# lukors/kanter_core

Hardware: AMD Instinct MI355X
Metric: node-Mpix/s on 4096x4096 f32x4, 32-node graph (higher is better)
Workload: dtype f32

## Files before the change

bindings/rust/kanter_core_amd_sys.rs:

```rust
#![allow(non_camel_case_types, dead_code)]
use std::os::raw::{c_char, c_void};

pub const KC_OK: i32 = 0;
pub const KC_ERR_GENERIC: i32 = 1;
pub const KC_ERR_CANCELED: i32 = 2;
pub const KC_ERR_IMAGE: i32 = 3;
pub const KC_ERR_INVALID_BUFFER_COUNT: i32 = 4;
pub const KC_ERR_INVALID_NODE_ID: i32 = 5;
pub const KC_ERR_INVALID_NODE_TYPE: i32 = 6;
pub const KC_ERR_INVALID_SLOT_ID: i32 = 7;
pub const KC_ERR_INVALID_SLOT_TYPE: i32 = 8;
pub const KC_ERR_INVALID_EDGE: i32 = 9;
pub const KC_ERR_NO_SLOT_DATA: i32 = 10;
pub const KC_ERR_SLOT_OCCUPIED: i32 = 11;
pub const KC_ERR_SLOT_NOT_OCCUPIED: i32 = 12;
pub const KC_ERR_UNABLE_TO_LOCK: i32 = 13;
pub const KC_ERR_NODE_PROCESSING: i32 = 14;
pub const KC_ERR_POISON: i32 = 15;
pub const KC_ERR_TRY_LOCK: i32 = 16;
pub const KC_ERR_NODE_DIRTY: i32 = 17;
pub const KC_ERR_IO: i32 = 18;
pub const KC_ERR_INVALID_NAME: i32 = 19;
pub const KC_ERR_HIP: i32 = 100;
pub const KC_ERR_NO_DEVICE: i32 = 101;
// ... 216 lines not shown
pub const KC_PARTITION_SPREAD: i32 = 1;
pub const KC_PARTITION_BANDS: i32 = 2;

pub const KC_PLAN_SINGLE: i32 = 0;
pub const KC_PLAN_BRANCHES: i32 = 1;
pub const KC_PLAN_BANDS: i32 = 2;

#[repr(C)] #[derive(Clone, Copy, Debug, PartialEq, Eq)]
pub struct KcBandRange {
    pub y0: i32,
    pub y1: i32,
}

pub const KC_KIND_SOURCE: i32 = 0;
pub const KC_KIND_REPLICATED: i32 = 1;
pub const KC_KIND_COMPUTE: i32 = 2;

#[repr(C)] #[derive(Clone, Copy, Debug, PartialEq, Eq)]
pub struct KcPlacement {
    pub node_id: u32,
    pub rank: i32,
    pub component: i32,
    pub kind: i32,
}

#[repr(C)] #[derive(Clone, Copy, Debug, PartialEq, Eq)]
pub struct KcTransfer {
    pub node_id: u32,
    pub slot_id: u32,
    pub src_rank: i32,
    pub dst_rank: i32,
    pub level: i32,
}

pub const KC_COMM_ID_BYTES: usize = 256;

#[repr(C)] #[derive(Clone, Copy, Debug, PartialEq, Eq)]
pub struct KcBandRows {
    pub node_id: u32,
    pub y0: i32,
    pub y1: i32,
    pub width: u32,
    pub height: u32,
}

#[link(name = "kanter_core_amd")]
extern "C" {
    pub fn kc_init(device_ordinal: i32) -> i32;
    pub fn kc_shutdown() -> i32;
    pub fn kc_is_initialized() -> i32;
    pub fn kc_set_stream(hip_stream: *mut c_void) -> i32;
    pub fn kc_get_stream() -> *mut c_void;
    pub fn kc_sync() -> i32;
    pub fn kc_last_error() -> *const c_char;
    pub fn kc_status_string(status: i32) -> *const c_char;
    pub fn kc_set_fusion(enabled: i32) -> i32;
    pub fn kc_get_fusion() -> i32;
    pub fn kc_set_resize_mode(mode: i32) -> i32;
    pub fn kc_get_resize_mode() -> i32;
    pub fn kc_set_cache_policy(mode: i32) -> i32;
    pub fn kc_get_cache_policy() -> i32;
    pub fn kc_set_option(name: *const c_char, value: i32) -> i32;
    pub fn kc_get_option(name: *const c_char, value: *mut i32) -> i32;
    pub fn kc_resize_upsample_plan(in_n: u32, out_n: u32, filter: i32, eligible: *mut i32, info: *mut i32, rows: *mut f32, cap: usize) -> i32;
    pub fn kc_resize_down2_plan(in_n: u32, out_n: u32, filter: i32, info: *mut i32, left_count: *mut u32, w: *mut f32, wcap: usize, vrec: *mut u32, vcap: usize, hw: *mut f32, hcap: usize) -> i32;
    pub fn kc_stats(bytes_in_use: *mut u64, bytes_cached: *mut u64, kernel_launches: *mut u64) -> i32;
    pub fn kc_stats_algorithmic_bytes(bytes: *mut u64) -> i32;
    pub fn kc_stats_counter(name: *const c_char, value: *mut u64) -> i32;
    pub fn kc_pool_trim() -> i32;
    pub fn kc_set_specialize(mode: i32, after: i32) -> i32;
    pub fn kc_get_specialize() -> i32;
    pub fn kc_specialize_wait() -> i32;
    pub fn kc_specialize_stats(kernels_compiled: *mut u64, compiles_failed: *mut u64, specialized_launches: *mut u64, compiles_pending: *mut u64) -> i32;
    pub fn kc_specialize_compile_check(words: *const u32, n_ops: u32, n_in: u32, start_src: i32, flat: i32, source: *mut c_char, cap: usize) -> i32;
    pub fn kc_specialize_compile_check_mask(words: *const u32, n_ops: u32, n_in: u32, start_src: i32, flat: i32, nt_mask: u32, source: *mut c_char, cap: usize) -> i32;
    pub fn kc_set_chain_quads(quads: i32) -> i32;
    pub fn kc_get_chain_quads() -> i32;
    pub fn kc_specialize_compile_check_upsample(words: *const u32, n_ops: u32, n_in: u32, start_src: i32, taps: u32, wide: i32, source: *mut c_char, cap: usize) -> i32;
    pub fn kc_kernel_cache_set_dir(dir: *const c_char) -> i32;
    pub fn kc_kernel_cache_stats(files_accepted: *mut u64, files_refused: *mut u64, files_written: *mut u64, kernels_loaded: *mut u64) -> i32;
    pub fn kc_kernel_cache_precompile(words: *const u32, n_ops: u32, n_in: u32, start_src: i32, flat: i32, nt_mask: u32, up_taps: u32, up_wide: i32, dir: *const c_char) -> i32;
    pub fn kc_specialize_reset() -> i32;
    pub fn kc_kernel_cache_precompile_packed(words: *const u32, n_ops: u32, n_in: u32, start_src: i32, flat: i32, nt_mask: u32, in_tiers: u32, dir: *const c_char) -> i32;
    pub fn kc_set_pack_sources(mode: i32) -> i32;
    pub fn kc_get_pack_sources() -> i32;
    pub fn kc_set_pack_budget_mb(mb: i32) -> i32;
    pub fn kc_get_pack_budget_mb() -> i32;
    pub fn kc_plane_alloc(width: u32, height: u32, out: *mut *mut KcPlane) -> i32;
    pub fn kc_plane_const(width: u32, height: u32, value: f32, out: *mut *mut KcPlane) -> i32;
    pub fn kc_plane_wrap(device_ptr: *mut c_void, width: u32, height: u32, pitch_bytes: usize, out: *mut *mut KcPlane) -> i32;
    pub fn kc_plane_retain(p: *mut KcPlane) -> i32;
    pub fn kc_plane_release(p: *mut KcPlane) -> i32;
    pub fn kc_plane_size(p: *const KcPlane, width: *mut u32, height: *mut u32) -> i32;
    pub fn kc_plane_is_const(p: *const KcPlane, is_const: *mut i32, value: *mut f32) -> i32;
    pub fn kc_plane_materialize(p: *mut KcPlane) -> i32;
    pub fn kc_plane_device_ptr(p: *mut KcPlane, device_ptr: *mut *mut c_void, pitch_bytes: *mut usize) -> i32;
    pub fn kc_plane_upload_f32(p: *mut KcPlane, host: *const f32, host_pitch_bytes: usize) -> i32;
    pub fn kc_plane_download_f32(p: *mut KcPlane, host: *mut f32, host_pitch_bytes: usize) -> i32;
    pub fn kc_image_gray(p: *mut KcPlane, out: *mut *mut KcImage) -> i32;
    pub fn kc_image_rgba(planes: *const *mut KcPlane, out: *mut *mut KcImage) -> i32;
    pub fn kc_image_retain(img: *mut KcImage) -> i32;
    pub fn kc_image_release(img: *mut KcImage) -> i32;
    pub fn kc_image_is_rgba(img: *const KcImage, is_rgba: *mut i32) -> i32;
    pub fn kc_image_size(img: *const KcImage, size: *mut KcSize) -> i32;
    pub fn kc_image_plane(img: *const KcImage, channel: i32, out: *mut *mut KcPlane) -> i32;
    pub fn kc_image_from_value(size: KcSize, value: f32, rgba: i32, out: *mut *mut KcImage) -> i32;
    pub fn kc_image_as_type(img: *const KcImage, rgba: i32, out: *mut *mut KcImage) -> i32;
    pub fn kc_image_materialize(img: *mut KcImage) -> i32;
    pub fn kc_image_from_u8(host: *const u8, width: u32, height: u32, channels: i32, out: *mut *mut KcImage) -> i32;
    pub fn kc_image_to_u8(img: *mut KcImage, srgb: i32, host_rgba8: *mut u8) -> i32;
    pub fn kc_u8_pipe_create(width: u32, height: u32, channels: i32, depth: i32, out: *mut *mut KcU8Pipe) -> i32;
    pub fn kc_u8_pipe_free(pipe: *mut KcU8Pipe) -> i32;
    pub fn kc_u8_pipe_buffers(pipe: *mut KcU8Pipe, slot: i32, host_in: *mut *mut u8, host_out: *mut *const u8) -> i32;
    pub fn kc_u8_pipe_upload(pipe: *mut KcU8Pipe, slot: i32, out: *mut *mut KcImage) -> i32;
    pub fn kc_u8_pipe_download(pipe: *mut KcU8Pipe, slot: i32, img: *mut KcImage, srgb: i32) -> i32;
    pub fn kc_u8_pipe_wait_download(pipe: *mut KcU8Pipe, slot: i32) -> i32;
    pub fn kc_image_from_f32(host_planes: *const *const f32, n_planes: i32, width: u32, height: u32, out: *mut *mut KcImage) -> i32;
    pub fn kc_image_to_f32(img: *mut KcImage, host_planes: *const *mut f32, n_planes: i32) -> i32;
    pub fn kc_device_image_validate(d: *const KcDeviceImage, extent_bytes: *mut usize) -> i32;
    pub fn kc_image_from_device(src: *const KcDeviceImage, flags: u32, hip_stream: *mut c_void, out: *mut *mut KcImage) -> i32;
    pub fn kc_image_to_device(img: *mut KcImage, dst: *const KcDeviceImage, flags: u32, hip_stream: *mut c_void) -> i32;
    pub fn kc_image_channel_stats(img: *mut KcImage, flags: u32, out: *mut KcChannelStats) -> i32;
    pub fn kc_bc_image_validate(d: *const KcBcImage, extent_bytes: *mut usize) -> i32;
    pub fn kc_bc1_punch_through_block(rgba: *const u8, ref_u8: u32, block: *mut u8) -> i32;
    pub fn kc_image_to_bc(img: *mut KcImage, format: i32, flags: u32, host: *mut u8, host_bytes: usize) -> i32;
    pub fn kc_image_to_bc_device(img: *mut KcImage, dst: *const KcBcImage, flags: u32, hip_stream: *mut c_void) -> i32;
    pub fn kc_mip_level_count(width: u32, height: u32, levels: *mut u32) -> i32;
    pub fn kc_preview_level(width: u32, height: u32, max_extent: u32, level: *mut u32, level_width: *mut u32, level_height: *mut u32) -> i32;
    pub fn kc_image_previews(r: *const KcPreviewRequest, count: u32, flags: u32, host: *mut u8, host_bytes: usize) -> i32;
    pub fn kc_image_previews_device(r: *const KcPreviewRequest, count: u32, flags: u32, device_ptr: *mut c_void, bytes: usize, hip_stream: *mut c_void) -> i32;
    pub fn kc_live_graph_buffer_previews(lg: *mut KcLiveGraph, node_ids: *const u32, slot_ids: *const u32, r: *const KcPreviewRequest, count: u32, flags: u32, host: *mut u8, host_bytes: usize) -> i32;
    pub fn kc_preview_plan(width: u32, height: u32, level: u32, x: u32, y: u32, rect_w: u32, rect_h: u32, out: *mut KcPreviewPlanInfo) -> i32;
    pub fn kc_mip_normal_texel(box_: *const f32, out: *mut f32) -> i32;
    pub fn kc_alpha_ref_threshold(ref_u8: u32, r: *mut f32) -> i32;
    pub fn kc_mip_coverage_target(width: u32, height: u32, covered0: u64, level: u32, target: *mut u64) -> i32;
    pub fn kc_mip_coverage_scale(v: f32, ref_u8: u32, s: *mut f32) -> i32;
    pub fn kc_image_mip_coverage_info(img: *mut KcImage, flags: u32, out: *mut KcMipCoverageLevel, cap: u32, count: *mut u32) -> i32;
    pub fn kc_mip_alpha_weight(a: f32, w: *mut f32) -> i32;
    pub fn kc_mip_alpha_texel(p: *const f32, w: f32, q: *mut f32, known: *mut i32) -> i32;
    pub fn kc_image_build_mips(img: *mut KcImage, flags: u32, levels: *mut *mut KcImage, cap: u32, count: *mut u32) -> i32;
    pub fn kc_bc_mip_layout(width: u32, height: u32, format: i32, levels: *mut u32, offsets: *mut usize, cap: u32, total_bytes: *mut usize) -> i32;
    pub fn kc_image_to_bc_mips(img: *mut KcImage, format: i32, flags: u32, host: *mut u8, host_bytes: usize) -> i32;
    pub fn kc_image_to_bc_mips_device(img: *mut KcImage, format: i32, flags: u32, device_ptr: *mut c_void, bytes: usize, hip_stream: *mut c_void) -> i32;
    pub fn kc_dds_header(width: u32, height: u32, format: i32, flags: u32, levels: u32, out: *mut u8, bytes: *mut usize) -> i32;
    pub fn kc_image_write_dds(img: *mut KcImage, path: *const c_char, format: i32, flags: u32, with_mips: i32) -> i32;
    pub fn kc_mip_unit_normal(rgb: *const f32, u: *mut f32) -> i32;
    pub fn kc_mip_roughness_texel(m: *const f32, r: f32, power: f32, d: *mut f32) -> i32;
    pub fn kc_image_build_roughness_mips(img: *mut KcImage, channel: u32, normals: *mut KcImage, power: f32, flags: u32, levels: *mut *mut KcImage, cap: u32, count: *mut u32) -> i32;
    pub fn kc_image_levels_to_bc_mips(levels: *mut *mut KcImage, count: u32, format: i32, flags: u32, host: *mut u8, host_bytes: usize) -> i32;
    pub fn kc_image_levels_write_dds(levels: *mut *mut KcImage, count: u32, path: *const c_char, format: i32, flags: u32) -> i32;
    pub fn kc_image_distance_field(img: *mut KcImage, channel: u32, ref_u8: u32, spread: u32, flags: u32, out: *mut *mut KcImage) -> i32;
    pub fn kc_sdf_texel(d2: u32, inside: i32, spread: u32, v: *mut f32) -> i32;
    pub fn kc_sdf_cap(spread: u32, cap: *mut u32) -> i32;
    pub fn kc_image_from_bc(host: *const u8, host_bytes: usize, width: u32, height: u32, format: i32, flags: u32, out: *mut *mut KcImage, undecoded_blocks: *mut u64) -> i32;
    pub fn kc_image_from_bc_device(src: *const KcBcImage, flags: u32, hip_stream: *mut c_void, out: *mut *mut KcImage, undecoded_blocks: *mut u64) -> i32;
    pub fn kc_image_bc_compare(img: *mut KcImage, blocks: *const KcBcImage, flags: u32, out: *mut KcBcError) -> i32;
    pub fn kc_image_bc_error(img: *mut KcImage, format: i32, flags: u32, out: *mut KcBcError) -> i32;
    pub fn kc_dds_parse(data: *const u8, bytes: usize, info: *mut KcDdsInfo) -> i32;
    pub fn kc_image_read_dds(path: *const c_char, level: u32, flags: u32, out: *mut *mut KcImage, info: *mut KcDdsInfo) -> i32;
    pub fn kc_image_read_png(path: *const c_char, out: *mut *mut KcImage) -> i32;
    pub fn kc_image_write_png(img: *mut KcImage, path: *const c_char) -> i32;
    pub fn kc_calculate_size(policy: i32, sizes: *const KcSize, n: i32, slot_index: i32, specific: KcSize, out: *mut KcSize) -> i32;
    pub fn kc_resize_image(src: *mut KcImage, size: KcSize, filter: i32, out: *mut *mut KcImage) -> i32;
    pub fn kc_resize_buffers(images: *const *mut KcImage, keys: *const KcEdge, n: i32, edges_sorted: *const KcEdge, n_edges: i32, policy: i32, policy_slot: u32, policy_size: KcSize, filter: i32, out: *mut *mut KcImage) -> i32;
    pub fn kc_mix_process(left: *mut KcImage, right: *mut KcImage, mix_type: i32, out: *mut *mut KcImage) -> i32;
    pub fn kc_separate_rgba_process(input: *mut KcImage, out: *mut *mut KcImage) -> i32;
// ... 87 lines not shown
```

include/kanter_core_amd.h:

```cpp
#ifndef KANTER_CORE_AMD_H
#define KANTER_CORE_AMD_H

#include <stddef.h>
#include <stdint.h>

#ifdef __cplusplus
extern "C" {
#endif

#define KC_API __attribute__((visibility("default")))

typedef enum kc_status {
    KC_OK = 0,
    KC_ERR_GENERIC = 1,
    KC_ERR_CANCELED = 2,
    KC_ERR_IMAGE = 3,
    KC_ERR_INVALID_BUFFER_COUNT = 4,
    KC_ERR_INVALID_NODE_ID = 5,
    KC_ERR_INVALID_NODE_TYPE = 6,
    KC_ERR_INVALID_SLOT_ID = 7,
    KC_ERR_INVALID_SLOT_TYPE = 8,
    KC_ERR_INVALID_EDGE = 9,
    KC_ERR_NO_SLOT_DATA = 10,
    KC_ERR_SLOT_OCCUPIED = 11,
// ... 12 lines not shown
    KC_ERR_UNSUPPORTED = 104
} kc_status;

typedef enum kc_mix_type { KC_MIX_ADD = 0, KC_MIX_SUBTRACT = 1, KC_MIX_MULTIPLY = 2, KC_MIX_DIVIDE = 3, KC_MIX_POW = 4 } kc_mix_type;
typedef enum kc_resize_filter { KC_FILTER_NEAREST = 0, KC_FILTER_TRIANGLE = 1, KC_FILTER_CATMULLROM = 2, KC_FILTER_GAUSSIAN = 3, KC_FILTER_LANCZOS3 = 4 } kc_resize_filter;
typedef enum kc_resize_policy { KC_POLICY_MOST_PIXELS = 0, KC_POLICY_LEAST_PIXELS = 1, KC_POLICY_LARGEST_AXES = 2, KC_POLICY_SMALLEST_AXES = 3, KC_POLICY_SPECIFIC_SLOT = 4, KC_POLICY_SPECIFIC_SIZE = 5 } kc_resize_policy;
typedef enum kc_node_type {
    KC_NODE_INPUT_GRAY = 0, KC_NODE_INPUT_RGBA = 1, KC_NODE_OUTPUT_GRAY = 2, KC_NODE_OUTPUT_RGBA = 3,
    KC_NODE_GRAPH = 4, KC_NODE_IMAGE = 5, KC_NODE_EMBED = 6, KC_NODE_WRITE = 7, KC_NODE_VALUE = 8,
    KC_NODE_MIX = 9, KC_NODE_HEIGHT_TO_NORMAL = 10, KC_NODE_SEPARATE_RGBA = 11, KC_NODE_COMBINE_RGBA = 12
} kc_node_type;
typedef enum kc_node_state { KC_STATE_CLEAN = 0, KC_STATE_DIRTY = 1, KC_STATE_REQUESTED = 2, KC_STATE_PRIORITISED = 3, KC_STATE_PROCESSING = 4, KC_STATE_PROCESSING_DIRTY = 5 } kc_node_state;
typedef enum kc_side { KC_SIDE_INPUT = 0, KC_SIDE_OUTPUT = 1 } kc_side;

typedef struct kc_plane kc_plane;
typedef struct kc_image kc_image;
typedef struct kc_node_graph kc_node_graph;
typedef struct kc_live_graph kc_live_graph;
typedef struct kc_tex_pro kc_tex_pro;
typedef struct kc_partition kc_partition;
typedef struct kc_u8_pipe kc_u8_pipe;

typedef struct kc_size { uint32_t width, height; } kc_size;
typedef struct kc_edge { uint32_t output_id, input_id, output_slot, input_slot; } kc_edge;

typedef struct kc_node_desc {
    uint32_t node_id;
    int32_t node_type;
    int32_t mix_type;
    float value;
    uint32_t embed_id;
    const char *text;
    const kc_node_graph *graph;
    int32_t resize_policy;
    uint32_t policy_slot;
    kc_size policy_size;
    int32_t resize_filter;
} kc_node_desc;

KC_API int kc_init(int device_ordinal);
KC_API int kc_shutdown(void);
KC_API int kc_is_initialized(void);
KC_API int kc_set_stream(void *hip_stream);
KC_API void *kc_get_stream(void);
KC_API int kc_sync(void);
KC_API const char *kc_last_error(void);
KC_API const char *kc_status_string(int status);
KC_API int kc_set_fusion(int enabled);
KC_API int kc_get_fusion(void);
KC_API int kc_set_resize_mode(int mode);
KC_API int kc_get_resize_mode(void);
KC_API int kc_set_cache_policy(int mode);
KC_API int kc_get_cache_policy(void);
KC_API int kc_set_option(const char *name, int value);
KC_API int kc_get_option(const char *name, int *value);
KC_API int kc_resize_upsample_plan(uint32_t in_n, uint32_t out_n, int filter, int *eligible, int32_t info[5], float *rows,
                                   size_t cap);
KC_API int kc_resize_down2_plan(uint32_t in_n, uint32_t out_n, int filter, int32_t info[5], uint32_t *left_count, float *w, size_t wcap,
                                uint32_t *vrec, size_t vcap, float *hw, size_t hcap);
KC_API int kc_stats(uint64_t *bytes_in_use, uint64_t *bytes_cached, uint64_t *kernel_launches);
KC_API int kc_stats_algorithmic_bytes(uint64_t *bytes);
KC_API int kc_stats_counter(const char *name, uint64_t *value);
KC_API int kc_pool_trim(void);
KC_API int kc_set_specialize(int mode, int after);
KC_API int kc_get_specialize(void);
KC_API int kc_specialize_wait(void);
KC_API int kc_specialize_stats(uint64_t *kernels_compiled, uint64_t *compiles_failed, uint64_t *specialized_launches,
                               uint64_t *compiles_pending);
KC_API int kc_specialize_compile_check(const uint32_t *words, uint32_t n_ops, uint32_t n_in, int start_src, int flat,
                                       char *source, size_t cap);
KC_API int kc_specialize_compile_check_mask(const uint32_t *words, uint32_t n_ops, uint32_t n_in, int start_src, int flat,
                                            uint32_t nt_mask, char *source, size_t cap);
KC_API int kc_set_chain_quads(int quads);
KC_API int kc_get_chain_quads(void);
KC_API int kc_specialize_compile_check_upsample(const uint32_t *words, uint32_t n_ops, uint32_t n_in, int start_src, uint32_t taps,
                                                int wide, char *source, size_t cap);
KC_API int kc_kernel_cache_set_dir(const char *dir);
KC_API int kc_kernel_cache_stats(uint64_t *files_accepted, uint64_t *files_refused, uint64_t *files_written, uint64_t *kernels_loaded);
KC_API int kc_kernel_cache_precompile(const uint32_t *words, uint32_t n_ops, uint32_t n_in, int start_src, int flat, uint32_t nt_mask,
                                      uint32_t up_taps, int up_wide, const char *dir);
KC_API int kc_specialize_reset(void);
KC_API int kc_kernel_cache_precompile_packed(const uint32_t *words, uint32_t n_ops, uint32_t n_in, int start_src, int flat,
                                             uint32_t nt_mask, uint32_t in_tiers, const char *dir);
KC_API int kc_set_pack_sources(int mode);
KC_API int kc_get_pack_sources(void);
KC_API int kc_set_pack_budget_mb(int mb);
KC_API int kc_get_pack_budget_mb(void);

KC_API int kc_plane_alloc(uint32_t width, uint32_t height, kc_plane **out);
KC_API int kc_plane_const(uint32_t width, uint32_t height, float value, kc_plane **out);
KC_API int kc_plane_wrap(void *device_ptr, uint32_t width, uint32_t height, size_t pitch_bytes, kc_plane **out);
KC_API int kc_plane_retain(kc_plane *p);
KC_API int kc_plane_release(kc_plane *p);
KC_API int kc_plane_size(const kc_plane *p, uint32_t *width, uint32_t *height);
KC_API int kc_plane_is_const(const kc_plane *p, int *is_const, float *value);
KC_API int kc_plane_materialize(kc_plane *p);
KC_API int kc_plane_device_ptr(kc_plane *p, void **device_ptr, size_t *pitch_bytes);
KC_API int kc_plane_upload_f32(kc_plane *p, const float *host, size_t host_pitch_bytes);
KC_API int kc_plane_download_f32(kc_plane *p, float *host, size_t host_pitch_bytes);

KC_API int kc_image_gray(kc_plane *p, kc_image **out);
KC_API int kc_image_rgba(kc_plane *const planes[4], kc_image **out);
KC_API int kc_image_retain(kc_image *img);
KC_API int kc_image_release(kc_image *img);
KC_API int kc_image_is_rgba(const kc_image *img, int *is_rgba);
KC_API int kc_image_size(const kc_image *img, kc_size *size);
KC_API int kc_image_plane(const kc_image *img, int channel, kc_plane **out);
KC_API int kc_image_from_value(kc_size size, float value, int rgba, kc_image **out);
KC_API int kc_image_as_type(const kc_image *img, int rgba, kc_image **out);
KC_API int kc_image_materialize(kc_image *img);
KC_API int kc_image_from_u8(const uint8_t *host, uint32_t width, uint32_t height, int channels, kc_image **out);
KC_API int kc_image_to_u8(kc_image *img, int srgb, uint8_t *host_rgba8);
KC_API int kc_u8_pipe_create(uint32_t width, uint32_t height, int channels, int depth, kc_u8_pipe **out);
KC_API int kc_u8_pipe_free(kc_u8_pipe *pipe);
KC_API int kc_u8_pipe_buffers(kc_u8_pipe *pipe, int slot, uint8_t **host_in, const uint8_t **host_out);
KC_API int kc_u8_pipe_upload(kc_u8_pipe *pipe, int slot, kc_image **out);
KC_API int kc_u8_pipe_download(kc_u8_pipe *pipe, int slot, kc_image *img, int srgb);
KC_API int kc_u8_pipe_wait_download(kc_u8_pipe *pipe, int slot);
KC_API int kc_image_from_f32(const float *const host_planes[], int n_planes, uint32_t width, uint32_t height, kc_image **out);
KC_API int kc_image_to_f32(kc_image *img, float *const host_planes[], int n_planes);
typedef enum kc_dtype { KC_DTYPE_U8 = 0, KC_DTYPE_U16 = 1, KC_DTYPE_F16 = 2, KC_DTYPE_BF16 = 3, KC_DTYPE_F32 = 4 } kc_dtype;
typedef enum kc_layout { KC_LAYOUT_INTERLEAVED = 0 , KC_LAYOUT_PLANAR = 1  } kc_layout;
typedef struct kc_device_image {
    void *ptr;
    uint32_t width, height;
    int32_t channels;
    int32_t dtype, layout;
    size_t row_pitch_bytes;
    size_t channel_pitch_bytes;
} kc_device_image;
#define KC_DEVICE_SRGB 1u
#define KC_DEVICE_GRAY 2u
KC_API int kc_device_image_validate(const kc_device_image *d, size_t *extent_bytes);
KC_API int kc_image_from_device(const kc_device_image *src, uint32_t flags, void *hip_stream, kc_image **out);
KC_API int kc_image_to_device(kc_image *img, const kc_device_image *dst, uint32_t flags, void *hip_stream);
#define KC_STATS_HISTOGRAM 1u
#define KC_STATS_SRGB 2u
typedef struct kc_channel_stats {
    uint32_t channels;
    uint32_t flags;
    uint64_t pixels;
    float min[4], max[4];
    uint64_t nan_count[4];
    uint64_t histogram[4][256];
} kc_channel_stats;
KC_API int kc_image_channel_stats(kc_image *img, uint32_t flags, kc_channel_stats *out);
typedef enum kc_bc_format { KC_BC1 = 1, KC_BC3 = 3, KC_BC4 = 4, KC_BC5 = 5, KC_BC6H = 95, KC_BC7 = 98 } kc_bc_format;
typedef struct kc_bc_image {
    void *ptr;
    uint32_t width, height;
    int32_t format;
    size_t row_pitch_bytes;
} kc_bc_image;
#define KC_BC_SRGB 1u
#define KC_BC_PUNCH_THROUGH 256u
#define KC_BC_PUNCH_THROUGH_REF(b) (256u | ((uint32_t)(b) << 24))
KC_API int kc_bc_image_validate(const kc_bc_image *d, size_t *extent_bytes);
KC_API int kc_bc1_punch_through_block(const uint8_t rgba[64], uint32_t ref_u8, uint8_t block[8]);
KC_API int kc_image_to_bc(kc_image *img, int format, uint32_t flags, uint8_t *host, size_t host_bytes);
KC_API int kc_image_to_bc_device(kc_image *img, const kc_bc_image *dst, uint32_t flags, void *hip_stream);
#define KC_MIP_PER_LEVEL 2u
#define KC_MIP_NORMALS 32u
#define KC_MIP_COVERAGE 64u
#define KC_MIP_COVERAGE_REF(b) (64u | ((uint32_t)(b) << 24))
#define KC_MIP_ALPHA_WEIGHT 128u
typedef struct kc_mip_coverage_level {
// ... 215 lines not shown
```

kanter_core_amd/__init__.py:

```python
from .api import (Edge, EmbeddedSlotDataId, LiveGraph, MixType, Node, NodeGraph, NodeId, NodeState, NodeType,
                  ResizeFilter, ResizePolicy, Side, Size, SlotData, SlotId, SlotImage, TexProError,
                  TextureProcessor, calculate_size, combine_rgba_process, get_stream, height_to_normal_process,
                  init, is_initialized, mix_process, resize_image, separate_rgba_process, set_fusion, set_stream,
                  shutdown, stats, sync, value_process, set_specialize, get_specialize, specialize_wait,
                  specialize_stats, specialize_compile_check, Partition, PartitionPolicy, NodeKind, set_resize_mode,
                  get_resize_mode, resize_upsample_plan, resize_down2_plan, stats_counter, specialize_compile_check_upsample, specialize_compile_check_mask, set_chain_quads, get_chain_quads, set_pack_sources, get_pack_sources, set_pack_budget_mb, get_pack_budget_mb, set_cache_policy, get_cache_policy, set_option, get_option, comm_unique_id, comm_init,
                  comm_destroy, comm_info, comm_stats, comm_transport, comm_gather_bands, PlanKind, pool_trim, kernel_cache_set_dir, kernel_cache_stats,
                  kernel_cache_precompile, specialize_reset, U8Pipe, device_image_desc, DEVICE_SRGB, DEVICE_GRAY,
                  ChannelStats, STATS_HISTOGRAM, STATS_SRGB, BC_SRGB, BC6H, BC7, BC_BLOCK_BYTES, BC_PUNCH_THROUGH, bc_punch_through_ref, bc1_punch_through_block,
                  MIP_PER_LEVEL, MIP_NORMALS, MIP_COVERAGE, MIP_ALPHA_WEIGHT, mip_alpha_weight, mip_alpha_texel, mip_coverage_ref, MipCoverageLevel, alpha_ref_threshold, mip_coverage_target, mip_coverage_scale, mip_normal_texel, mip_unit_normal, mip_roughness_texel, levels_to_bc_mips, write_dds_levels, mip_level_count, bc_mip_layout, dds_header, BC_GRAY, BC_ALL_MODES, BcError, DdsInfo, dds_parse, preview_level,
                  PREVIEW_SRGB, PreviewPlan, preview_plan, previews, previews_torch, SDF_WRAP, SDF_MAX_SPREAD, sdf_cap, sdf_texel)

__all__ = [n for n in dir() if not n.startswith("_")]
```

kanter_core_amd/_abi.py:

```python
import ctypes as C


KC_OK = 0
KC_ERR_GENERIC = 1
KC_ERR_CANCELED = 2
KC_ERR_IMAGE = 3
KC_ERR_INVALID_BUFFER_COUNT = 4
KC_ERR_INVALID_NODE_ID = 5
KC_ERR_INVALID_NODE_TYPE = 6
KC_ERR_INVALID_SLOT_ID = 7
KC_ERR_INVALID_SLOT_TYPE = 8
KC_ERR_INVALID_EDGE = 9
KC_ERR_NO_SLOT_DATA = 10
KC_ERR_SLOT_OCCUPIED = 11
KC_ERR_SLOT_NOT_OCCUPIED = 12
KC_ERR_UNABLE_TO_LOCK = 13
KC_ERR_NODE_PROCESSING = 14
KC_ERR_POISON = 15
KC_ERR_TRY_LOCK = 16
KC_ERR_NODE_DIRTY = 17
KC_ERR_IO = 18
KC_ERR_INVALID_NAME = 19
KC_ERR_HIP = 100
KC_ERR_NO_DEVICE = 101
# ... 234 lines not shown


class kc_band_range(C.Structure):
    _fields_ = [
        ("y0", C.c_int32),
        ("y1", C.c_int32),
    ]


KC_KIND_SOURCE = 0
KC_KIND_REPLICATED = 1
KC_KIND_COMPUTE = 2


class kc_placement(C.Structure):
    _fields_ = [
        ("node_id", C.c_uint32),
        ("rank", C.c_int32),
        ("component", C.c_int32),
        ("kind", C.c_int32),
    ]


class kc_transfer(C.Structure):
    _fields_ = [
        ("node_id", C.c_uint32),
        ("slot_id", C.c_uint32),
        ("src_rank", C.c_int32),
        ("dst_rank", C.c_int32),
        ("level", C.c_int32),
    ]


KC_COMM_ID_BYTES = 256


class kc_band_rows(C.Structure):
    _fields_ = [
        ("node_id", C.c_uint32),
        ("y0", C.c_int32),
        ("y1", C.c_int32),
        ("width", C.c_uint32),
        ("height", C.c_uint32),
    ]


SIGNATURES = {
    "kc_init": (C.c_int, [C.c_int]),
    "kc_shutdown": (C.c_int, []),
    "kc_is_initialized": (C.c_int, []),
    "kc_set_stream": (C.c_int, [C.c_void_p]),
    "kc_get_stream": (C.c_void_p, []),
    "kc_sync": (C.c_int, []),
    "kc_last_error": (C.c_char_p, []),
    "kc_status_string": (C.c_char_p, [C.c_int]),
    "kc_set_fusion": (C.c_int, [C.c_int]),
    "kc_get_fusion": (C.c_int, []),
    "kc_set_resize_mode": (C.c_int, [C.c_int]),
    "kc_get_resize_mode": (C.c_int, []),
    "kc_set_cache_policy": (C.c_int, [C.c_int]),
    "kc_get_cache_policy": (C.c_int, []),
    "kc_set_option": (C.c_int, [C.c_char_p, C.c_int]),
    "kc_get_option": (C.c_int, [C.c_char_p, C.POINTER(C.c_int)]),
    "kc_resize_upsample_plan": (C.c_int, [C.c_uint32, C.c_uint32, C.c_int, C.POINTER(C.c_int), C.POINTER(C.c_int32), C.c_void_p, C.c_size_t]),
    "kc_resize_down2_plan": (C.c_int, [C.c_uint32, C.c_uint32, C.c_int, C.POINTER(C.c_int32), C.POINTER(C.c_uint32), C.c_void_p, C.c_size_t, C.POINTER(C.c_uint32), C.c_size_t, C.c_void_p, C.c_size_t]),
    "kc_stats": (C.c_int, [C.POINTER(C.c_uint64), C.POINTER(C.c_uint64), C.POINTER(C.c_uint64)]),
    "kc_stats_algorithmic_bytes": (C.c_int, [C.POINTER(C.c_uint64)]),
    "kc_stats_counter": (C.c_int, [C.c_char_p, C.POINTER(C.c_uint64)]),
    "kc_pool_trim": (C.c_int, []),
    "kc_set_specialize": (C.c_int, [C.c_int, C.c_int]),
    "kc_get_specialize": (C.c_int, []),
    "kc_specialize_wait": (C.c_int, []),
    "kc_specialize_stats": (C.c_int, [C.POINTER(C.c_uint64), C.POINTER(C.c_uint64), C.POINTER(C.c_uint64), C.POINTER(C.c_uint64)]),
    "kc_specialize_compile_check": (C.c_int, [C.POINTER(C.c_uint32), C.c_uint32, C.c_uint32, C.c_int, C.c_int, C.c_char_p, C.c_size_t]),
    "kc_specialize_compile_check_mask": (C.c_int, [C.POINTER(C.c_uint32), C.c_uint32, C.c_uint32, C.c_int, C.c_int, C.c_uint32, C.c_char_p, C.c_size_t]),
    "kc_set_chain_quads": (C.c_int, [C.c_int]),
    "kc_get_chain_quads": (C.c_int, []),
    "kc_specialize_compile_check_upsample": (C.c_int, [C.POINTER(C.c_uint32), C.c_uint32, C.c_uint32, C.c_int, C.c_uint32, C.c_int, C.c_char_p, C.c_size_t]),
    "kc_kernel_cache_set_dir": (C.c_int, [C.c_char_p]),
    "kc_kernel_cache_stats": (C.c_int, [C.POINTER(C.c_uint64), C.POINTER(C.c_uint64), C.POINTER(C.c_uint64), C.POINTER(C.c_uint64)]),
    "kc_kernel_cache_precompile": (C.c_int, [C.POINTER(C.c_uint32), C.c_uint32, C.c_uint32, C.c_int, C.c_int, C.c_uint32, C.c_uint32, C.c_int, C.c_char_p]),
    "kc_specialize_reset": (C.c_int, []),
    "kc_kernel_cache_precompile_packed": (C.c_int, [C.POINTER(C.c_uint32), C.c_uint32, C.c_uint32, C.c_int, C.c_int, C.c_uint32, C.c_uint32, C.c_char_p]),
    "kc_set_pack_sources": (C.c_int, [C.c_int]),
    "kc_get_pack_sources": (C.c_int, []),
    "kc_set_pack_budget_mb": (C.c_int, [C.c_int]),
    "kc_get_pack_budget_mb": (C.c_int, []),
    "kc_plane_alloc": (C.c_int, [C.c_uint32, C.c_uint32, C.POINTER(C.c_void_p)]),
    "kc_plane_const": (C.c_int, [C.c_uint32, C.c_uint32, C.c_float, C.POINTER(C.c_void_p)]),
    "kc_plane_wrap": (C.c_int, [C.c_void_p, C.c_uint32, C.c_uint32, C.c_size_t, C.POINTER(C.c_void_p)]),
    "kc_plane_retain": (C.c_int, [C.c_void_p]),
    "kc_plane_release": (C.c_int, [C.c_void_p]),
    "kc_plane_size": (C.c_int, [C.c_void_p, C.POINTER(C.c_uint32), C.POINTER(C.c_uint32)]),
    "kc_plane_is_const": (C.c_int, [C.c_void_p, C.POINTER(C.c_int), C.c_void_p]),
    "kc_plane_materialize": (C.c_int, [C.c_void_p]),
    "kc_plane_device_ptr": (C.c_int, [C.c_void_p, C.POINTER(C.c_void_p), C.POINTER(C.c_size_t)]),
    "kc_plane_upload_f32": (C.c_int, [C.c_void_p, C.c_void_p, C.c_size_t]),
    "kc_plane_download_f32": (C.c_int, [C.c_void_p, C.c_void_p, C.c_size_t]),
    "kc_image_gray": (C.c_int, [C.c_void_p, C.POINTER(C.c_void_p)]),
    "kc_image_rgba": (C.c_int, [C.POINTER(C.c_void_p), C.POINTER(C.c_void_p)]),
    "kc_image_retain": (C.c_int, [C.c_void_p]),
    "kc_image_release": (C.c_int, [C.c_void_p]),
    "kc_image_is_rgba": (C.c_int, [C.c_void_p, C.POINTER(C.c_int)]),
    "kc_image_size": (C.c_int, [C.c_void_p, C.POINTER(kc_size)]),
    "kc_image_plane": (C.c_int, [C.c_void_p, C.c_int, C.POINTER(C.c_void_p)]),
    "kc_image_from_value": (C.c_int, [kc_size, C.c_float, C.c_int, C.POINTER(C.c_void_p)]),
    "kc_image_as_type": (C.c_int, [C.c_void_p, C.c_int, C.POINTER(C.c_void_p)]),
    "kc_image_materialize": (C.c_int, [C.c_void_p]),
    "kc_image_from_u8": (C.c_int, [C.c_void_p, C.c_uint32, C.c_uint32, C.c_int, C.POINTER(C.c_void_p)]),
    "kc_image_to_u8": (C.c_int, [C.c_void_p, C.c_int, C.c_void_p]),
    "kc_u8_pipe_create": (C.c_int, [C.c_uint32, C.c_uint32, C.c_int, C.c_int, C.POINTER(C.c_void_p)]),
    "kc_u8_pipe_free": (C.c_int, [C.c_void_p]),
    "kc_u8_pipe_buffers": (C.c_int, [C.c_void_p, C.c_int, C.POINTER(C.c_void_p), C.POINTER(C.c_void_p)]),
    "kc_u8_pipe_upload": (C.c_int, [C.c_void_p, C.c_int, C.POINTER(C.c_void_p)]),
    "kc_u8_pipe_download": (C.c_int, [C.c_void_p, C.c_int, C.c_void_p, C.c_int]),
    "kc_u8_pipe_wait_download": (C.c_int, [C.c_void_p, C.c_int]),
    "kc_image_from_f32": (C.c_int, [C.POINTER(C.c_void_p), C.c_int, C.c_uint32, C.c_uint32, C.POINTER(C.c_void_p)]),
    "kc_image_to_f32": (C.c_int, [C.c_void_p, C.POINTER(C.c_void_p), C.c_int]),
    "kc_device_image_validate": (C.c_int, [C.POINTER(kc_device_image), C.POINTER(C.c_size_t)]),
    "kc_image_from_device": (C.c_int, [C.POINTER(kc_device_image), C.c_uint32, C.c_void_p, C.POINTER(C.c_void_p)]),
    "kc_image_to_device": (C.c_int, [C.c_void_p, C.POINTER(kc_device_image), C.c_uint32, C.c_void_p]),
    "kc_image_channel_stats": (C.c_int, [C.c_void_p, C.c_uint32, C.POINTER(kc_channel_stats)]),
    "kc_bc_image_validate": (C.c_int, [C.POINTER(kc_bc_image), C.POINTER(C.c_size_t)]),
    "kc_bc1_punch_through_block": (C.c_int, [C.c_void_p, C.c_uint32, C.c_void_p]),
    "kc_image_to_bc": (C.c_int, [C.c_void_p, C.c_int, C.c_uint32, C.c_void_p, C.c_size_t]),
    "kc_image_to_bc_device": (C.c_int, [C.c_void_p, C.POINTER(kc_bc_image), C.c_uint32, C.c_void_p]),
    "kc_mip_level_count": (C.c_int, [C.c_uint32, C.c_uint32, C.POINTER(C.c_uint32)]),
    "kc_preview_level": (C.c_int, [C.c_uint32, C.c_uint32, C.c_uint32, C.POINTER(C.c_uint32), C.POINTER(C.c_uint32), C.POINTER(C.c_uint32)]),
    "kc_image_previews": (C.c_int, [C.POINTER(kc_preview_request), C.c_uint32, C.c_uint32, C.c_void_p, C.c_size_t]),
    "kc_image_previews_device": (C.c_int, [C.POINTER(kc_preview_request), C.c_uint32, C.c_uint32, C.c_void_p, C.c_size_t, C.c_void_p]),
    "kc_live_graph_buffer_previews": (C.c_int, [C.c_void_p, C.POINTER(C.c_uint32), C.POINTER(C.c_uint32), C.POINTER(kc_preview_request), C.c_uint32, C.c_uint32, C.c_void_p, C.c_size_t]),
    "kc_preview_plan": (C.c_int, [C.c_uint32, C.c_uint32, C.c_uint32, C.c_uint32, C.c_uint32, C.c_uint32, C.c_uint32, C.POINTER(kc_preview_plan_info)]),
    "kc_mip_normal_texel": (C.c_int, [C.c_void_p, C.c_void_p]),
    "kc_alpha_ref_threshold": (C.c_int, [C.c_uint32, C.c_void_p]),
    "kc_mip_coverage_target": (C.c_int, [C.c_uint32, C.c_uint32, C.c_uint64, C.c_uint32, C.POINTER(C.c_uint64)]),
    "kc_mip_coverage_scale": (C.c_int, [C.c_float, C.c_uint32, C.c_void_p]),
    "kc_image_mip_coverage_info": (C.c_int, [C.c_void_p, C.c_uint32, C.POINTER(kc_mip_coverage_level), C.c_uint32, C.POINTER(C.c_uint32)]),
    "kc_mip_alpha_weight": (C.c_int, [C.c_float, C.c_void_p]),
    "kc_mip_alpha_texel": (C.c_int, [C.c_void_p, C.c_float, C.c_void_p, C.POINTER(C.c_int)]),
    "kc_image_build_mips": (C.c_int, [C.c_void_p, C.c_uint32, C.POINTER(C.c_void_p), C.c_uint32, C.POINTER(C.c_uint32)]),
    "kc_bc_mip_layout": (C.c_int, [C.c_uint32, C.c_uint32, C.c_int, C.POINTER(C.c_uint32), C.POINTER(C.c_size_t), C.c_uint32, C.POINTER(C.c_size_t)]),
    "kc_image_to_bc_mips": (C.c_int, [C.c_void_p, C.c_int, C.c_uint32, C.c_void_p, C.c_size_t]),
    "kc_image_to_bc_mips_device": (C.c_int, [C.c_void_p, C.c_int, C.c_uint32, C.c_void_p, C.c_size_t, C.c_void_p]),
    "kc_dds_header": (C.c_int, [C.c_uint32, C.c_uint32, C.c_int, C.c_uint32, C.c_uint32, C.c_void_p, C.POINTER(C.c_size_t)]),
    "kc_image_write_dds": (C.c_int, [C.c_void_p, C.c_char_p, C.c_int, C.c_uint32, C.c_int]),
    "kc_mip_unit_normal": (C.c_int, [C.c_void_p, C.c_void_p]),
    "kc_mip_roughness_texel": (C.c_int, [C.c_void_p, C.c_float, C.c_float, C.c_void_p]),
    "kc_image_build_roughness_mips": (C.c_int, [C.c_void_p, C.c_uint32, C.c_void_p, C.c_float, C.c_uint32, C.POINTER(C.c_void_p), C.c_uint32, C.POINTER(C.c_uint32)]),
    "kc_image_levels_to_bc_mips": (C.c_int, [C.POINTER(C.c_void_p), C.c_uint32, C.c_int, C.c_uint32, C.c_void_p, C.c_size_t]),
    "kc_image_levels_write_dds": (C.c_int, [C.POINTER(C.c_void_p), C.c_uint32, C.c_char_p, C.c_int, C.c_uint32]),
    "kc_image_distance_field": (C.c_int, [C.c_void_p, C.c_uint32, C.c_uint32, C.c_uint32, C.c_uint32, C.POINTER(C.c_void_p)]),
    "kc_sdf_texel": (C.c_int, [C.c_uint32, C.c_int, C.c_uint32, C.c_void_p]),
    "kc_sdf_cap": (C.c_int, [C.c_uint32, C.POINTER(C.c_uint32)]),
    "kc_image_from_bc": (C.c_int, [C.c_void_p, C.c_size_t, C.c_uint32, C.c_uint32, C.c_int, C.c_uint32, C.POINTER(C.c_void_p), C.POINTER(C.c_uint64)]),
    "kc_image_from_bc_device": (C.c_int, [C.POINTER(kc_bc_image), C.c_uint32, C.c_void_p, C.POINTER(C.c_void_p), C.POINTER(C.c_uint64)]),
    "kc_image_bc_compare": (C.c_int, [C.c_void_p, C.POINTER(kc_bc_image), C.c_uint32, C.POINTER(kc_bc_error)]),
    "kc_image_bc_error": (C.c_int, [C.c_void_p, C.c_int, C.c_uint32, C.POINTER(kc_bc_error)]),
    "kc_dds_parse": (C.c_int, [C.c_void_p, C.c_size_t, C.POINTER(kc_dds_info)]),
    "kc_image_read_dds": (C.c_int, [C.c_char_p, C.c_uint32, C.c_uint32, C.POINTER(C.c_void_p), C.POINTER(kc_dds_info)]),
    "kc_image_read_png": (C.c_int, [C.c_char_p, C.POINTER(C.c_void_p)]),
    "kc_image_write_png": (C.c_int, [C.c_void_p, C.c_char_p]),
    "kc_calculate_size": (C.c_int, [C.c_int, C.POINTER(kc_size), C.c_int, C.c_int, kc_size, C.POINTER(kc_size)]),
    "kc_resize_image": (C.c_int, [C.c_void_p, kc_size, C.c_int, C.POINTER(C.c_void_p)]),
    "kc_resize_buffers": (C.c_int, [C.POINTER(C.c_void_p), C.POINTER(kc_edge), C.c_int, C.POINTER(kc_edge), C.c_int, C.c_int, C.c_uint32, kc_size, C.c_int, C.POINTER(C.c_void_p)]),
    "kc_mix_process": (C.c_int, [C.c_void_p, C.c_void_p, C.c_int, C.POINTER(C.c_void_p)]),
    "kc_separate_rgba_process": (C.c_int, [C.c_void_p, C.POINTER(C.c_void_p)]),
# ... 87 lines not shown
```

kanter_core_amd/api.py:

```python
import collections
import ctypes as C
import os

import numpy as np

from . import _abi, _lib
from ._lib import kc_edge, kc_node_desc, kc_size

_VARIANT_NAMES = {"KC_ERR_POISON": "PoisonError", "KC_ERR_TRY_LOCK": "TryLockError", "KC_ERR_INVALID_ARG": "InvalidArgument"}
_ERROR_NAMES = {v: _VARIANT_NAMES.get(k, k[len("KC_ERR_"):].title().replace("_", ""))
                for k, v in vars(_abi).items() if k.startswith("KC_ERR_")}


class TexProError(Exception):

    def __init__(self, code, detail=""):
        self.code = code
        self.kind = _ERROR_NAMES.get(code, "Unknown")
        L = _lib.load()
        msg = L.kc_status_string(code).decode()
        super().__init__("%s: %s%s" % (self.kind, msg, (" (" + detail + ")") if detail else ""))

    def __eq__(self, other):
        return isinstance(other, TexProError) and other.code == self.code
# ... 106 lines not shown


def get_option(name):
    v = C.c_int()
    _check(_lib.load().kc_get_option(name.encode(), C.byref(v)))
    return v.value


def resize_upsample_plan(in_n, out_n, filter=None):
    import numpy as np
    L = _lib.load()
    f = ResizeFilter.default() if filter is None else filter
    ok = C.c_int(0)
    info = (C.c_int32 * 5)()
    _check(L.kc_resize_upsample_plan(int(in_n), int(out_n), int(f), C.byref(ok), info, None, 0))
    if not ok.value:
        return None
    ratio, taps, off, b_lo, b_hi = (int(v) for v in info)
    rows = np.zeros(((ratio + b_lo + b_hi), taps), np.float32)
    _check(L.kc_resize_upsample_plan(int(in_n), int(out_n), int(f), C.byref(ok), info,
                                     rows.ctypes.data_as(C.POINTER(C.c_float)), rows.size))
    return dict(ratio=ratio, taps=taps, off=off, b_lo=b_lo, b_hi=b_hi, rows=rows)


def resize_down2_plan(in_n, out_n, filter=None):
    import numpy as np
    L = _lib.load()
    f = ResizeFilter.default() if filter is None else filter
    info = (C.c_int32 * 5)()
    _check(L.kc_resize_down2_plan(int(in_n), int(out_n), int(f), info, None, None, 0, None, 0, None, 0))
    stride, nc, hstride, tile_w, min_count = (int(v) for v in info)
    groups = (out_n + 3) // 4
    lc = np.zeros(2 * out_n, np.uint32)
    w = np.zeros((out_n, stride), np.float32)
    vrec = np.zeros((groups, max(nc, 1), 72), np.uint32)
    hw = np.zeros((out_n, max(hstride, 1)), np.float32)
    _check(L.kc_resize_down2_plan(int(in_n), int(out_n), int(f), info, lc.ctypes.data_as(C.POINTER(C.c_uint32)),
                                  w.ctypes.data_as(C.POINTER(C.c_float)), w.size,
                                  vrec.ctypes.data_as(C.POINTER(C.c_uint32)), vrec.size if nc else 0,
                                  hw.ctypes.data_as(C.POINTER(C.c_float)), hw.size if hstride else 0))
    return dict(stride=stride, nc=nc, hstride=hstride, tile_w=tile_w, min_count=min_count, left=lc[:out_n].copy(),
                count=lc[out_n:].copy(), w=w, vrec=vrec if nc else None, hw=hw if hstride else None)


def set_specialize(mode, after=0):
    _check(_lib.load().kc_set_specialize(int(mode), int(after)))


def get_specialize():
    return _lib.load().kc_get_specialize()


def specialize_wait():
    _check(_lib.load().kc_specialize_wait())


def specialize_stats():
    v = [C.c_uint64() for _ in range(4)]
    _check(_lib.load().kc_specialize_stats(*[C.byref(x) for x in v]))
    return dict(zip(("kernels_compiled", "compiles_failed", "specialized_launches", "compiles_pending"), [x.value for x in v]))


def specialize_compile_check(words, n_in, start_src=0, flat=True):
    arr = (C.c_uint32 * len(words))(*words)
    buf = C.create_string_buffer(1 << 16)
    _check(_lib.load().kc_specialize_compile_check(arr, len(words), int(n_in), int(start_src), int(bool(flat)), buf, len(buf)))
    return buf.value.decode()


def specialize_compile_check_mask(words, n_in, nt_mask, start_src=0, flat=True):
    arr = (C.c_uint32 * len(words))(*words)
    buf = C.create_string_buffer(1 << 17)
    _check(_lib.load().kc_specialize_compile_check_mask(arr, len(words), int(n_in), int(start_src), int(bool(flat)), int(nt_mask),
                                                        buf, len(buf)))
    return buf.value.decode()


def set_chain_quads(quads):
    _check(_lib.load().kc_set_chain_quads(int(quads)))


def get_chain_quads():
    return _lib.load().kc_get_chain_quads()


def set_pack_sources(mode):
    _check(_lib.load().kc_set_pack_sources(int(mode)))


def get_pack_sources():
    return _lib.load().kc_get_pack_sources()


def set_pack_budget_mb(mb):
    _check(_lib.load().kc_set_pack_budget_mb(int(mb)))


def get_pack_budget_mb():
    return _lib.load().kc_get_pack_budget_mb()


def specialize_compile_check_upsample(words, n_in, start_src=0, taps=3, wide=True):
    arr = (C.c_uint32 * len(words))(*words)
    buf = C.create_string_buffer(1 << 17)
    _check(_lib.load().kc_specialize_compile_check_upsample(arr, len(words), int(n_in), int(start_src), int(taps), int(bool(wide)),
                                                            buf, len(buf)))
    return buf.value.decode()


def stats():
    a, b, c = C.c_uint64(), C.c_uint64(), C.c_uint64()
    _check(_lib.load().kc_stats(C.byref(a), C.byref(b), C.byref(c)))
    d = C.c_uint64()
    _check(_lib.load().kc_stats_algorithmic_bytes(C.byref(d)))
    return {"bytes_in_use": a.value, "bytes_cached": b.value, "kernel_launches": c.value, "algorithmic_bytes": d.value}


def kernel_cache_set_dir(path):
    _check(_lib.load().kc_kernel_cache_set_dir(None if path is None else str(path).encode()))


def kernel_cache_stats():
    v = [C.c_uint64() for _ in range(4)]
    _check(_lib.load().kc_kernel_cache_stats(*[C.byref(x) for x in v]))
    return dict(zip(("files_accepted", "files_refused", "files_written", "kernels_loaded"), (x.value for x in v)))


def kernel_cache_precompile(words, n_in, start_src, flat, nt_mask, directory, up_taps=0, up_wide=False, in_tiers=0):
    arr = (C.c_uint32 * len(words))(*words)
    if in_tiers:
        if up_taps:
            raise ValueError("packed inputs: plain chain programs only")
        _check(_lib.load().kc_kernel_cache_precompile_packed(arr, len(words), int(n_in), int(start_src), int(bool(flat)), int(nt_mask),
                                                             int(in_tiers), str(directory).encode()))
        return
    _check(_lib.load().kc_kernel_cache_precompile(arr, len(words), int(n_in), int(start_src), int(bool(flat)), int(nt_mask),
                                                  int(up_taps), int(bool(up_wide)), str(directory).encode()))


def specialize_reset():
    _check(_lib.load().kc_specialize_reset())


def pool_trim():
    _check(_lib.load().kc_pool_trim())


def stats_counter(name):
    v = C.c_uint64()
    _check(_lib.load().kc_stats_counter(name.encode(), C.byref(v)))
    return v.value


class NodeId(int):
    """NodeId(u32), src/node_graph.rs:592-607"""


class SlotId(int):
    """SlotId(u32), src/node_graph.rs:609-624"""


class EmbeddedSlotDataId(int):
    """src/node/embed.rs:13-14"""


class Size:
# ... 1426 lines not shown
```

kanter_core_amd/build.py:

```python
import os
import subprocess
import sys
from concurrent.futures import ThreadPoolExecutor

HERE = os.path.dirname(os.path.abspath(__file__))
CSRC = os.path.join(HERE, "csrc")
OBJ = os.path.join(HERE, "csrc", "build")
LIB = os.path.join(HERE, "libkanter_core_amd.so")
SOURCES = ["chain.hip", "upsample.hip", "resize_tile.hip", "resize_down.hip", "h2n.hip", "u8.hip", "chain1.hip", "down2.hip", "runtime.cpp",
           "ops.cpp", "resize.cpp", "graph.cpp", "json.cpp", "png.cpp", "specialize.cpp", "partition.cpp", "bands.cpp", "comm.cpp", "replay.cpp",
           "u8pipe.cpp", "devimage.hip", "devimage.cpp", "stats.hip", "stats.cpp", "bc.hip", "bc1a.hip", "bc7.hip", "bc6h.hip", "bc.cpp", "mip.hip", "mip_normals.hip", "mip_roughness.hip", "mip_alpha.hip", "mip_coverage.hip", "mip.cpp", "mip_export.cpp", "preview.hip", "preview.cpp", "sdf.hip", "sdf.cpp", "bc_decode.hip",
           "bc_decode.cpp", "bc_modes.hip", "chain_pack.hip", "chain_pack.cpp",
           "c_api.cpp"]
HEADERS = ["kc_internal.hpp", "kc_runtime.hpp", "chain_program.h", "chain_pack.h", "preview_walk.h", "mip_steps.h", os.path.join("..", "..", "include", "kanter_core_amd.h"), "pow_positive.inc",
           "srgb_thresholds.inc", "streaming.h", "bc_blocks.h", "bc_modes.h", "upsample.h", "upsample_chain.inc", "chain_apply.inc", "chain_interp.inc", "resample.inc"]
JIT_TEXTS = [("kJitChainProgramH", "chain_program.h"), ("kJitPowPositiveInc", "pow_positive.inc"), ("kJitUpsampleH", "upsample.h"),
             ("kJitUpsampleChainInc", "upsample_chain.inc"), ("kJitChainPackH", "chain_pack.h")]

FLAGS = ["--offload-arch=gfx950", "-O3", "-std=c++17", "-fPIC", "-fvisibility=hidden", "-fno-fast-math",
         "-ffp-contract=off", "-fhip-fp32-correctly-rounded-divide-sqrt", "-Wall", "-Wno-unused-result"]
DEVICE_FLAGS = ["-mllvm", "-structurizecfg-skip-uniform-regions=1"]
if os.environ.get("KC_HOST_PROFILE"):
    FLAGS = FLAGS + ["-DKC_HOST_PROFILE"]
if os.environ.get("KC_HOST_SAMPLE"):
    FLAGS = FLAGS + ["-DKC_HOST_SAMPLE", "-fno-omit-frame-pointer"]


def _hipcc():
    for cand in (os.environ.get("HIPCC"), "/opt/rocm/bin/hipcc", "hipcc"):
        if cand and (os.path.isabs(cand) and os.path.exists(cand) or not os.path.isabs(cand)):
            return cand
    return "hipcc"


def _stale(target, deps):
    if not os.path.exists(target):
        return True
    t = os.path.getmtime(target)
    return any(os.path.getmtime(d) > t for d in deps)


def object_name(src):
    stem = os.path.splitext(src)[0]
    if src.endswith(".hip") and stem + ".cpp" in SOURCES:
        stem += "_kernels"
    return stem + ".o"


def _write_jit_texts():
    out = os.path.join(OBJ, "jit_texts.cpp")
    parts = ["// generated by kanter_core_amd/build.py from csrc/chain_program.h and csrc/pow_positive.inc -- do not edit\n",
             "namespace kc {\n"]
    for name, fn in JIT_TEXTS:
        with open(os.path.join(CSRC, fn)) as f:
            text = f.read()
        assert ')KCJIT"' not in text
        parts.append('extern const char %s[];\nconst char %s[] = R"KCJIT(\n%s)KCJIT";\n' % (name, name, text))
    parts.append("}  // namespace kc\n")
    new = "".join(parts)
    old = open(out).read() if os.path.exists(out) else None
    if new != old:
        with open(out, "w") as f:
            f.write(new)
    return out


def build(force=False, verbose=False):
    os.makedirs(OBJ, exist_ok=True)
    hipcc = _hipcc()
    hdrs = [os.path.join(CSRC, h) for h in HEADERS]
    jobs = []
    objs = []
    jit = _write_jit_texts()
    jit_o = os.path.join(OBJ, "jit_texts.o")
    objs.append(jit_o)
    if force or _stale(jit_o, [jit]):
        jobs.append([hipcc] + FLAGS + ["-c", jit, "-o", jit_o])
    for src in SOURCES:
        s = os.path.join(CSRC, src)
        o = os.path.join(OBJ, object_name(src))
        objs.append(o)
        if force or _stale(o, [s] + hdrs):
            cmd = [hipcc] + FLAGS + (DEVICE_FLAGS + ["-x", "hip"] if src.endswith(".hip") else []) + ["-c", s, "-o", o]
            jobs.append(cmd)

    def run(cmd):
        if verbose:
            print(" ".join(cmd), flush=True)
        r = subprocess.run(cmd, stdout=subprocess.PIPE, stderr=subprocess.STDOUT, text=True)
        if r.returncode != 0:
            raise RuntimeError("hipcc failed:\n%s\n%s" % (" ".join(cmd), r.stdout))
        return r.stdout

    with ThreadPoolExecutor(max_workers=4) as ex:
        for out in ex.map(run, jobs):
            if verbose and out.strip():
                print(out)
    if force or jobs or _stale(LIB, objs):
        run([hipcc, "--offload-arch=gfx950", "-shared", "-fPIC", "-o", LIB] + objs + ["-lz", "-ldl"])
    populate_kernel_cache(verbose=verbose)
    return LIB


MANIFEST = os.path.join(HERE, "baseline_programs.jsonl")
KERNEL_CACHE = os.path.join(HERE, "kernel_cache")


def populate_kernel_cache(force=False, verbose=False):
    import ctypes as C
    import hashlib
    import json
    if not os.path.exists(MANIFEST) or not os.path.exists(LIB):
        return 0
    with open(MANIFEST) as f:
        text = f.read()
    entries = [json.loads(line) for line in text.splitlines() if line.strip()]
    st = os.stat(LIB)
    stamp = hashlib.sha256(("%s|%d|%d" % (text, st.st_mtime_ns, st.st_size)).encode()).hexdigest()
    stamp_file = os.path.join(KERNEL_CACHE, ".stamp")
    if not force and os.path.exists(stamp_file) and open(stamp_file).read() == stamp:
        return len(entries)
    os.makedirs(KERNEL_CACHE, exist_ok=True)
    for old in os.listdir(KERNEL_CACHE):
        if old.endswith(".kcco"):
            os.remove(os.path.join(KERNEL_CACHE, old))
    L = C.CDLL(LIB)
    L.kc_kernel_cache_precompile.argtypes = [C.POINTER(C.c_uint32), C.c_uint32, C.c_uint32, C.c_int, C.c_int, C.c_uint32, C.c_uint32,
                                             C.c_int, C.c_char_p]
    L.kc_kernel_cache_precompile.restype = C.c_int
    L.kc_kernel_cache_precompile_packed.argtypes = [C.POINTER(C.c_uint32), C.c_uint32, C.c_uint32, C.c_int, C.c_int, C.c_uint32, C.c_uint32,
                                                    C.c_char_p]
    L.kc_kernel_cache_precompile_packed.restype = C.c_int
    L.kc_last_error.restype = C.c_char_p

    def one(e):
        words = (C.c_uint32 * len(e["words"]))(*e["words"])
        if e.get("in_tiers"):
            rc = L.kc_kernel_cache_precompile_packed(words, len(e["words"]), e["n_in"], e["start_src"], e["flat"], e["nt_mask"],
                                                     e["in_tiers"], KERNEL_CACHE.encode())
        else:
            rc = L.kc_kernel_cache_precompile(words, len(e["words"]), e["n_in"], e["start_src"], e["flat"], e["nt_mask"], e["up_taps"],
                                              e["up_wide"], KERNEL_CACHE.encode())
        if rc != 0:
            raise RuntimeError("pre-compiling %s failed (%d): %s" % (e.get("name"), rc, (L.kc_last_error() or b"").decode(errors="replace")))
        if verbose:
            print("pre-compiled", e.get("name"), flush=True)

    with ThreadPoolExecutor(max_workers=4) as ex:
        list(ex.map(one, entries))
    with open(stamp_file, "w") as f:
        f.write(stamp)
    return len(entries)


if __name__ == "__main__":
    print(build(force="--force" in sys.argv, verbose=True))
```

kanter_core_amd/csrc/c_api.cpp:

```cpp
#include <algorithm>
#include <cctype>
#include <climits>
#include <cstdio>
#include <cstdlib>
#include <cstring>
#include <fstream>
#include <sstream>

#include "kc_runtime.hpp"

namespace kc {
const std::string &last_error();
}
using namespace kc;

#define KC_ARG(cond)                                         \
    do {                                                     \
        if (!(cond)) {                                       \
            set_error("invalid argument: " #cond);           \
            return KC_ERR_INVALID_ARG;                       \
        }                                                    \
    } while (0)

typedef std::lock_guard<std::recursive_mutex> Lock;
// ... 347 lines not shown

int kc_specialize_compile_check_mask(const uint32_t *words, uint32_t n_ops, uint32_t n_in, int start_src, int flat, uint32_t nt_mask,
                                     char *source, size_t cap)
try {
    KC_ARG(words && n_ops >= 1 && n_ops <= (uint32_t)KC_CHAIN_MAX_OPS && n_in <= (uint32_t)KC_CHAIN_MAX_IN);
    KC_ARG(start_src >= -1 && start_src < (int)n_in);
    ChainProgram P;
    std::memset(&P, 0, sizeof P);
    P.n_ops = n_ops;
    P.n_in = n_in;
    P.start_src = start_src;
    P.rows = flat ? 1u : 2u;
    P.row_units = 1;
    P.nt_mask = nt_mask;
    for (uint32_t i = 0; i < n_ops; ++i) {
        const uint32_t from = (words[i] >> 8) & 0xffu, level = words[i] >> 16;
        KC_ARG((words[i] & 0xffu) <= CH_SAVE_LOAD && (from <= n_in || (from == (uint32_t)KC_CHAIN_SRC_SAVED && (words[i] & 0xffu) != CH_SAVE_LOAD)));
        KC_ARG(level < (uint32_t)KC_CHAIN_MAX_SAVED && (level == 0 || from == (uint32_t)KC_CHAIN_SRC_SAVED || (words[i] & 0xffu) == CH_SAVE_LOAD));
        ((i & 1u) ? P.step[0][i / 2].b : P.step[0][i / 2].a).word = words[i];
    }
    if (source && cap) {
        const std::string src = specialize_source(P);
        std::snprintf(source, cap, "%s", src.c_str());
    }
    std::string log;
    int s = specialize_compile_only(P, &log);
    if (s != KC_OK) set_error("specialised chain kernel did not compile: " + log);
    return s;
}
KC_CATCH

int kc_set_chain_quads(int quads)
try {
    const int s = specialize_set_chain_quads(quads);
    if (s != KC_OK) set_error("kc_set_chain_quads accepts 0, 1, 2 or 4");
    return s;
}
KC_CATCH

int kc_get_chain_quads(void)
try {
    return specialize_get_chain_quads();
}
catch (...) {
    return 0;
}

int kc_kernel_cache_set_dir(const char *dir)
try {
    Lock lk(ctx().mu);
    return kernel_cache_set_dir(dir);
}
KC_CATCH

int kc_kernel_cache_stats(uint64_t *hits, uint64_t *rejected, uint64_t *written, uint64_t *kernels_loaded)
try {
    kernel_cache_stats(hits, rejected, written, kernels_loaded);
    return KC_OK;
}
KC_CATCH

int kc_kernel_cache_precompile(const uint32_t *words, uint32_t n_ops, uint32_t n_in, int start_src, int flat, uint32_t nt_mask,
                               uint32_t up_taps, int up_wide, const char *dir)
try {
    KC_ARG(words && dir);
    std::string log;
    const int s = kernel_cache_precompile(words, n_ops, n_in, start_src, flat != 0, nt_mask, 0, up_taps, up_wide != 0, dir, &log);
    if (s != KC_OK) set_error("kernel cache: " + log);
    return s;
}
KC_CATCH

int kc_kernel_cache_precompile_packed(const uint32_t *words, uint32_t n_ops, uint32_t n_in, int start_src, int flat, uint32_t nt_mask,
                                      uint32_t in_tiers, const char *dir)
try {
    KC_ARG(words && dir);
    std::string log = "in_tiers: two bits per input plane, 0 to 2, flat programs only";
    const int s = kernel_cache_precompile(words, n_ops, n_in, start_src, flat != 0, nt_mask, in_tiers, 0, false, dir, &log);
    if (s != KC_OK) set_error("kernel cache: " + log);
    return s;
}
KC_CATCH

int kc_set_pack_sources(int mode)
try {
    Lock lk(ctx().mu);
    if (mode < 0 || mode > 2) {
        set_error("kc_set_pack_sources accepts 0, 1 or 2");
        return KC_ERR_INVALID_ARG;
    }
    ctx().pack_sources = mode;
    return KC_OK;
}
KC_CATCH

int kc_get_pack_sources(void)
try {
    return ctx().pack_sources;
}
catch (...) {
    return 0;
}

int kc_set_pack_budget_mb(int mb)
try {
    Lock lk(ctx().mu);
    if (mb < 0) {
        set_error("kc_set_pack_budget_mb accepts 0 and up");
        return KC_ERR_INVALID_ARG;
    }
    ctx().pack_budget_mb = mb;
    return KC_OK;
}
KC_CATCH

int kc_get_pack_budget_mb(void)
try {
    return ctx().pack_budget_mb;
}
catch (...) {
    return 0;
}

int kc_specialize_reset(void)
try {
    Lock lk(ctx().mu);
    if (ctx().stream) (void)hipStreamSynchronize(ctx().stream);
    const int mode = specialize_get_mode();
    specialize_shutdown();
    (void)mode;
    return KC_OK;
}
KC_CATCH

int kc_specialize_compile_check_upsample(const uint32_t *words, uint32_t n_ops, uint32_t n_in, int start_src, uint32_t taps, int wide,
                                         char *source, size_t cap)
try {
    KC_ARG(words && n_ops >= 1 && n_ops <= (uint32_t)KC_CHAIN_MAX_OPS && n_in >= 1 && n_in <= (uint32_t)KC_CHAIN_INTERP_IN);
    KC_ARG(start_src >= -1 && start_src < (int)n_in && (taps == 1 || taps == 3));
    ChainProgram P;
    std::memset(&P, 0, sizeof P);
    P.n_ops = n_ops;
    P.n_in = n_in;
    P.start_src = start_src;
    for (uint32_t i = 0; i < n_ops; ++i) {
        const uint32_t from = words[i] >> 8, code = words[i] & 0xffu;
        KC_ARG(code <= CH_MUL_INV && from <= n_in && code != CH_DIV_L && code != CH_DIV_R && code != CH_POW_L && code != CH_POW_R);
        ((i & 1u) ? P.step[0][i / 2].b : P.step[0][i / 2].a).word = words[i];
    }
    UpsampleArgs U{};
    U.H.taps = U.V.taps = taps;
    U.tile_w = wide ? 1024u : 256u;
    if (source && cap) {
        const std::string src = specialize_source(P, &U);
        std::snprintf(source, cap, "%s", src.c_str());
    }
    std::string log;
    int s = specialize_compile_only(P, &log, &U);
    if (s != KC_OK) set_error("specialised up-sampling kernel did not compile: " + log);
    return s;
}
KC_CATCH

int kc_stats(uint64_t *in_use, uint64_t *cached, uint64_t *launches)
try {
    Context &c = ctx();
// ... 1559 lines not shown
```

kanter_core_amd/csrc/kc_internal.hpp:

```cpp
#pragma once

#include <hip/hip_runtime.h>

#include <atomic>
#include <cstdint>
#include <map>
#include <memory>
#include <mutex>
#include <string>
#include <vector>

#include "../../include/kanter_core_amd.h"
#include "preview_walk.h"

namespace kc {

#include "chain_program.h"
#include "upsample.h"

struct Options {
    int chain1, replay, join, wide, fusion, down2, down2_by_rows, poly2, poly2_min_ratio, resize_mode, resize_tile_w, resize_tile_h;
    int poly_rows, poly2_xcd, down2_xcd, h2n_tiled, cache_policy, cache_budget_mb, nt_force, chain_unroll, max_blocks, tune_cap;
    int upload_ring, link_gbps, hbm_gbps;
};
Options option_defaults();
const Options &options();

struct TapsDev {
    const uint32_t *left;
    const uint32_t *count;
    const float *w;
    uint32_t stride;
};

struct Operand {
    const float *ptr;
    uint32_t pitch;
    float c;
};

struct ChainVariant {
    int k = -1, u = 0, mode = 0;
    bool nt = false;
};
hipError_t launch_chain(const ChainProgram &p, int batch, int mode, int max_blocks, int unroll, hipStream_t s, ChainVariant *var);
inline uint32_t chain_op_word(uint8_t code, int src) { return (uint32_t)code | ((uint32_t)(src + 1) << 8); }
hipError_t launch_fill(float *dst, uint32_t pitch_floats, uint32_t w, uint32_t h, float v, hipStream_t s);
struct Chain1Args {
    const float *start[KC_CHAIN_MAX_BATCH], *operand[KC_CHAIN_MAX_BATCH];
    float *out[KC_CHAIN_MAX_BATCH];
    uint32_t start_pitch[KC_CHAIN_MAX_BATCH], operand_pitch[KC_CHAIN_MAX_BATCH], out_pitch[KC_CHAIN_MAX_BATCH];
    float start_c[KC_CHAIN_MAX_BATCH], operand_c[KC_CHAIN_MAX_BATCH], c[KC_CHAIN_MAX_BATCH];
    uint32_t row_units, rows;
};
hipError_t launch_chain1(const Chain1Args &a, int batch, int code, unsigned nt, hipStream_t s, unsigned *launched_nt);
constexpr uint32_t KC_RESIZE_REG_TAPS = 8;
inline size_t resize_lds_bytes(uint32_t tile_h, uint32_t ncp, uint32_t v_stride, uint32_t tile_w, uint32_t h_stride)
{
    const size_t row = h_stride > KC_RESIZE_REG_TAPS ? (size_t)ncp + (ncp >> 5) + 1u : ncp;
    size_t n = (size_t)tile_h * row + 8u + 2u * tile_h + (size_t)tile_h * v_stride;
    if (h_stride > KC_RESIZE_REG_TAPS) n += 2u * tile_w + (size_t)tile_w * h_stride;
    return n * sizeof(float);
}
#define KC_DOWN_ROW_FLOATS 265u
inline size_t resize_down_lds_bytes(uint32_t tile_h, uint32_t ncp, uint32_t tile_w, uint32_t h_stride)
{
    (void)ncp;
    return ((size_t)tile_h * KC_DOWN_ROW_FLOATS + 2u * tile_w + (size_t)tile_w * (h_stride | 1u)) * sizeof(float);
}
struct ResizePlanes {
    const float *src[4];
    float *dst[4];
    uint32_t spitch[4], dpitch[4];
};
constexpr uint32_t KC_DOWN2_REC = 72, KC_DOWN2_MAX_CHUNKS = 4, KC_DOWN2_SLOTS = 256 + 32;
struct Down2Args {
    const uint32_t *vrec;
    const uint32_t *hleft, *hcount, *strips;
    const float *hw;
    uint32_t nc, hstride;
    uint32_t tile_w, dw, dh;
    uint32_t xcd_per, n_tiles, gy, gy_magic;
    uint32_t by_rows;
};
inline uint32_t down2_cols_per_lane(uint32_t weight_quads) { return weight_quads <= 3 ? 3u : weight_quads == 4 ? 2u : 1u; }
struct XcdOrder {
    uint32_t per, n, gy, magic;
};
inline XcdOrder xcd_order(uint32_t gx, uint32_t gy, bool want)
{
    XcdOrder o{ 0, 0, 0, 0 };
    if (!want || gy < 2) return o;
    const uint64_t n = (uint64_t)gx * gy, magic = ((1ull << 32) + gy - 1) / gy;
    if (n >= (1u << 24) || n * (magic * gy - (1ull << 32)) >= (1ull << 32)) return o;
    o.per = (uint32_t)((n + 7) / 8);
    o.n = (uint32_t)n;
    o.gy = gy;
    o.magic = (uint32_t)magic;
    return o;
}
// ... 299 lines not shown
```

kanter_core_amd/csrc/kc_runtime.hpp:

```cpp
#pragma once

#include <cstring>
#include <deque>
#include <set>
#include <tuple>
#include <type_traits>
#include <unordered_map>
#include <unordered_set>

#include "kc_internal.hpp"

namespace kc {
struct Chain;
struct ChainLink;
}

namespace kc {
#if defined(__SANITIZE_ADDRESS__) || defined(__SANITIZE_THREAD__)
#define KC_NO_OBJECT_POOL 1
#elif defined(__has_feature)
#if __has_feature(address_sanitizer) || __has_feature(thread_sanitizer)
#define KC_NO_OBJECT_POOL 1
#endif
#endif
// ... 346 lines not shown
    uint32_t k, sw, sh, fused;
    bool nt;
    uint32_t last() const { return k + (fused ? fused : 1u); }
};
std::vector<MipStep> mip_plan(uint32_t w, uint32_t h, uint32_t L, bool per_level, uint32_t in0, uint32_t in_below, uint32_t out_planes,
                              const Options &o = options());
int mip_level_count(uint32_t w, uint32_t h, uint32_t *levels);
int preview_level(uint32_t w, uint32_t h, uint32_t max_extent, uint32_t *level, uint32_t *pw, uint32_t *ph);
float mip_const_fold(float c);
void mip_normal_texel(const float box[3], float out[3]);
int image_build_mips(kc_image *img, uint32_t flags, kc_image **levels, uint32_t cap, uint32_t *count);
void mip_unit_normal(const float rgb[3], float u[3]);
float mip_roughness_texel(const float m[3], float r, float power);
int image_build_roughness_mips(kc_image *img, uint32_t channel, kc_image *normals, float power, uint32_t flags, kc_image **levels, uint32_t cap,
                               uint32_t *count);
float mip_alpha_weight(float a);
bool mip_alpha_texel(const float p[3], float w, float q[3]);
int mip_check_alpha_flags(uint32_t flags, const char *who);
constexpr uint32_t kCoverageFlagBits = KC_MIP_COVERAGE | 0xff000000u;
float alpha_ref_threshold(uint32_t ref_u8);
int mip_coverage_target(uint32_t w, uint32_t h, uint64_t covered0, uint32_t level, uint64_t *target);
float mip_coverage_scale(float v, uint32_t ref_u8);
int mip_check_coverage_flags(uint32_t flags, const char *who);
int image_mip_coverage_info(kc_image *img, uint32_t flags, kc_mip_coverage_level *out, uint32_t cap, uint32_t *count);
int bc_mip_layout(uint32_t w, uint32_t h, int format, uint32_t *levels, size_t *offsets, uint32_t cap, size_t *total_bytes);
int image_to_bc_mips(kc_image *img, int format, uint32_t flags, uint8_t *host, size_t host_bytes);
int image_to_bc_mips_device(kc_image *img, int format, uint32_t flags, void *device_ptr, size_t bytes, void *hip_stream);
int dds_header(uint32_t w, uint32_t h, int format, uint32_t flags, uint32_t levels, uint8_t *out, size_t *bytes);
int image_write_dds(kc_image *img, const char *path, int format, uint32_t flags, int with_mips);
int image_levels_to_bc_mips(kc_image *const *levels, uint32_t count, int format, uint32_t flags, uint8_t *host, size_t host_bytes, const char *who);
int image_levels_write_dds(kc_image *const *levels, uint32_t count, const char *path, int format, uint32_t flags);
int preview_plan(uint32_t w, uint32_t h, uint32_t level, uint32_t x, uint32_t y, uint32_t rect_w, uint32_t rect_h, kc_preview_plan_info *out);
int preview_check(const kc_preview_request *r, uint32_t count, uint32_t flags, const void *out, size_t out_bytes, bool images_named, const char *who);
int image_previews(const kc_preview_request *r, kc_image *const *imgs, uint32_t count, uint32_t flags, uint8_t *host, size_t host_bytes, const char *who);
int image_previews_device(const kc_preview_request *r, uint32_t count, uint32_t flags, void *device_ptr, size_t bytes, void *hip_stream);
void preview_release();
int image_channel_stats(kc_image *img, uint32_t flags, kc_channel_stats *out);
uint32_t quant_u8_host(float v);
int stats_buffers(size_t partials_bytes);
void channel_stats_release();
uint32_t sdf_cap(uint32_t spread);
float sdf_texel(uint32_t d2, bool inside, uint32_t spread);
int image_distance_field(kc_image *img, uint32_t channel, uint32_t ref_u8, uint32_t spread, uint32_t flags, kc_image **out);
int calculate_size(int policy, const kc_size *sizes, int n, int slot_index, kc_size specific, kc_size *out);
int mix_process(kc_image *left, kc_image *right, int mix_type, kc_image **out);
int separate_process(kc_image *in, kc_image *out[4]);
int combine_process(kc_image *const in[4], kc_image **out);
int value_process(float v, kc_image **out);
int height_to_normal_process(kc_image *in, kc_image **out);
int height_to_normal_band(kc_image *in_with_halo, uint32_t full_h, kc_image **out);

int build_taps_host(uint32_t in_n, uint32_t out_n, int filter, TapsHost &t);
int resize_image(kc_image *src, kc_size size, int filter, kc_image **out);
int resize_force(kc_plane *p);
int resize_planes_band(kc_plane *const *srcs, int n, int32_t src_y0, uint32_t src_h_full, kc_size dst_full, int32_t a, int32_t b,
                       int filter, kc_plane **outs);
int resize_force_many(kc_plane *const *planes, int n);
int chain_resize_launch(const ChainProgram &P, int batch, int mode, kc_plane *const *sampled, bool *launched);

hipError_t launch_chain_specialized(const ChainProgram &P, int batch, hipStream_t s, bool *launched, uint32_t *nt_mask, uint32_t *quads = nullptr);
uint32_t cache_policy_mask(uint64_t in_bytes, uint64_t out_bytes, uint32_t n_resident, const Options &o = options());
uint32_t chain_cache_policy(const uint32_t *refs, uint32_t n, uint64_t stream_bytes, uint64_t out_bytes);
hipError_t chain_dispatch(ChainProgram &P, int batch, int mode, uint32_t w, uint32_t h, size_t out_pitch_bytes,
                          kc_plane *const (*src)[KC_CHAIN_MAX_IN] = nullptr, const uint32_t *refs = nullptr, uint64_t *packed_saved = nullptr);
uint32_t pack_chain_inputs(const ChainProgram &P, int batch, kc_plane *const (*src)[KC_CHAIN_MAX_IN], const uint32_t *refs, uint32_t w, uint32_t h);
void plane_shadow_drop(kc_plane *p, bool never_again);
uint32_t pack_bytes_per_quad(uint32_t tier);
bool chain_pack_program_ok(const ChainProgram &P);
hipError_t launch_upsample_chain_specialized(const ChainProgram &P, int batch, const UpsampleArgs &U, hipStream_t s, bool *launched);
int specialize_set_mode(int mode, int after);
int specialize_get_mode();
int specialize_set_chain_quads(int quads);
int specialize_get_chain_quads();
void specialize_wait();
void specialize_stats(uint64_t *compiled, uint64_t *failed, uint64_t *launches, uint64_t *pending);
std::string specialize_last_log();
void specialize_shutdown();
std::string specialize_source(const ChainProgram &P, const UpsampleArgs *U = nullptr);
int specialize_compile_only(const ChainProgram &P, std::string *log, const UpsampleArgs *U = nullptr);
int kernel_cache_set_dir(const char *dir);
void kernel_cache_stats(uint64_t *hits, uint64_t *rejected, uint64_t *written, uint64_t *kernels_loaded);
bool kernel_cache_populated();
int kernel_cache_precompile(const uint32_t *words, uint32_t n_ops, uint32_t n_in, int32_t start_src, bool flat, uint32_t nt_mask, uint32_t in_tiers,
                            uint32_t up_taps, bool up_wide, const char *dir, std::string *log);

int u8_pipe_create(uint32_t w, uint32_t h, int channels, int depth, kc_u8_pipe **out);
int u8_pipe_free(kc_u8_pipe *p);
int u8_pipe_buffers(kc_u8_pipe *p, int slot, uint8_t **host_in, const uint8_t **host_out);
int u8_pipe_upload(kc_u8_pipe *p, int slot, kc_image **out);
int u8_pipe_download(kc_u8_pipe *p, int slot, kc_image *img, bool srgb);
int u8_pipe_wait_download(kc_u8_pipe *p, int slot);

int png_read(const std::string &path, std::vector<uint8_t> &px, uint32_t &w, uint32_t &h, int &channels);
int png_write_rgba8(const std::string &path, const uint8_t *px, uint32_t w, uint32_t h);

struct NodeGraph;

struct Node {
    uint32_t node_id = 0;
    int type = KC_NODE_VALUE;
    int mix_type = KC_MIX_ADD;
    float value = 0.0f;
    uint32_t embed_id = 0;
    std::string text;
    std::shared_ptr<NodeGraph> graph;
    int policy = KC_POLICY_MOST_PIXELS;
    uint32_t policy_slot = 0;
    kc_size policy_size{ 0, 0 };
    int filter = KC_FILTER_TRIANGLE;

    bool is_input() const { return type == KC_NODE_INPUT_GRAY || type == KC_NODE_INPUT_RGBA; }
    bool is_output() const { return type == KC_NODE_OUTPUT_GRAY || type == KC_NODE_OUTPUT_RGBA; }
    bool is_source() const { return type == KC_NODE_EMBED || type == KC_NODE_IMAGE || is_input(); }
};

enum SlotType { SLOT_GRAY = 0, SLOT_RGBA = 1, SLOT_GRAY_OR_RGBA = 2 };
struct Slot {
    std::string name;
    uint32_t slot_id;
    int slot_type;
};

struct GraphIndex {
    uint64_t version = ~0ull;
    size_t n_nodes = 0, n_edges = 0;
    std::unordered_map<uint32_t, uint32_t> node_pos;
    std::unordered_map<uint32_t, std::vector<kc_edge>> in_edges;
    std::unordered_map<uint32_t, std::vector<kc_edge>> out_edges;
};

struct NodeGraph {
    std::vector<Node> nodes;
    std::vector<kc_edge> edges;
    uint32_t node_id_counter = 0;
    uint64_t version = 0;
    mutable GraphIndex idx;

    void touch() { ++version; }
    const GraphIndex &index() const;
    bool index_is_current() const;
    void appended_node(bool index_was_current);
    void appended_edge(bool index_was_current);
    void erased_edge(const kc_edge &e, bool index_was_current);
    const std::vector<kc_edge> &edges_into(uint32_t id) const;
    const std::vector<kc_edge> &edges_out_of(uint32_t id) const;

    const Node *find(uint32_t id) const;
    Node *find(uint32_t id);
    uint32_t new_id();
    int add_node(Node n, uint32_t *id);
    int add_node_with_id(Node n);
    int connect(uint32_t on, uint32_t in, uint32_t os, uint32_t is);
    int try_connect(uint32_t on, uint32_t in, uint32_t os, uint32_t is);
    int remove_edge(kc_edge e);
    int remove_node(uint32_t id, std::vector<kc_edge> *removed);
    int disconnect_slot(uint32_t id, int side, uint32_t slot, std::vector<kc_edge> *removed);
    std::vector<uint32_t> get_children(uint32_t id) const;
    std::vector<uint32_t> get_children_recursive(uint32_t id) const;
    std::vector<uint32_t> get_parents(uint32_t id) const;
    std::vector<uint32_t> output_ids() const;
    int rename_output_node(uint32_t id, const std::string &new_name, std::string *old_name);
    std::vector<Slot> input_slots_of_graph() const;
    std::vector<Slot> output_slots_of_graph() const;
};

std::vector<Slot> node_input_slots(const Node &n, bool *unimplemented = nullptr);
std::vector<Slot> node_output_slots(const Node &n, bool *unimplemented = nullptr);
// ... 182 lines not shown
```

kanter_core_amd/csrc/replay.cpp:

```cpp
#include "kc_runtime.hpp"

using namespace kc;

struct kc_live_graph::ReplayEntry {
    uint32_t root = 0;
    uint64_t ghash = 0;
    std::vector<std::pair<uint32_t, int>> pre_state;
    struct Held {
        uint32_t node, slot;
        kc_image *img;
    };
    std::vector<Held> pre_slots;
    std::vector<EmbeddedSlotData> embedded;
    std::vector<std::pair<uint32_t, int>> post_state;
    std::vector<uint32_t> dropped;
    std::vector<uint32_t> changed_ids;
    std::vector<ReplayLaunch> launches;
    uint32_t w = 0, h = 0;
    uint32_t root_slot = 0;
    int n_planes = 0;
    int out_l[4] = { -1, -1, -1, -1 };
    int out_b[4] = { -1, -1, -1, -1 };
    float cval[4] = { 0, 0, 0, 0 };

    ~ReplayEntry()
    {
        for (auto &h : pre_slots) image_release(h.img);
        for (auto &em : embedded) image_release(em.image);
    }
};

namespace kc {

static uint64_t mix64(uint64_t h, uint64_t v)
{
    h ^= v + 0x9E3779B97F4A7C15ull + (h << 6) + (h >> 2);
    return h * 0xBF58476D1CE4E5B9ull;
}

static uint64_t graph_content_hash(const NodeGraph &g)
{
    uint64_t h = 0x243F6A8885A308D3ull;
    h = mix64(h, g.nodes.size());
    for (auto &n : g.nodes) {
        uint32_t vbits;
        std::memcpy(&vbits, &n.value, 4);
        h = mix64(h, ((uint64_t)n.node_id << 32) | (uint32_t)n.type);
        h = mix64(h, ((uint64_t)(uint32_t)n.mix_type << 32) | vbits);
        h = mix64(h, ((uint64_t)n.embed_id << 32) | (uint32_t)n.policy);
        h = mix64(h, ((uint64_t)n.policy_slot << 32) | (uint32_t)n.filter);
        h = mix64(h, ((uint64_t)n.policy_size.width << 32) | n.policy_size.height);
    }
    h = mix64(h, g.edges.size());
    for (auto &e : g.edges) {
        h = mix64(h, ((uint64_t)e.output_id << 32) | e.input_id);
        h = mix64(h, ((uint64_t)e.output_slot << 32) | e.input_slot);
    }
    return h;
}

static bool recordable_type(int t)
{
    return t == KC_NODE_MIX || t == KC_NODE_VALUE || t == KC_NODE_COMBINE_RGBA || t == KC_NODE_SEPARATE_RGBA ||
           t == KC_NODE_OUTPUT_GRAY || t == KC_NODE_OUTPUT_RGBA || t == KC_NODE_EMBED;
}

static size_t slot_count_except(const kc_live_graph &lg, uint32_t node)
{
    size_t n = 0;
    for (auto &kv : lg.slot_datas)
        if (kv.first != node) n += kv.second.size();
    return n;
}

int replay_try(kc_live_graph &lg, uint32_t id, bool *hit)
{
    *hit = false;
    const kc_live_graph::ReplayEntry *e = lg.replay;
    if (!e || e->root != id || lg.use_cache || lg.auto_update || !options().fusion || !options().replay) return KC_OK;
    if (e->pre_state.size() != lg.node_state.size()) return KC_OK;
    for (auto &ps : e->pre_state) {
        auto it = lg.node_state.find(ps.first);
        if (it == lg.node_state.end() || it->second != ps.second) return KC_OK;
    }
    if (slot_count_except(lg, id) != e->pre_slots.size()) return KC_OK;
    for (auto &h : e->pre_slots) {
        const SlotData *sd = lg.find_slot(h.node, h.slot);
        if (!sd || sd->image != h.img) return KC_OK;
    }
    if (lg.embedded.size() != e->embedded.size()) return KC_OK;
    for (size_t i = 0; i < e->embedded.size(); ++i) {
        const EmbeddedSlotData &a = lg.embedded[i], &b = e->embedded[i];
        if (a.image != b.image || a.slot_data_id != b.slot_data_id || a.slot_id != b.slot_id || a.full_h != b.full_h || a.band_y0 != b.band_y0)
            return KC_OK;
    }
    if (graph_content_hash(lg.g) != e->ghash) return KC_OK;

    Context &c = ctx();
    std::vector<kc_plane *> outs(e->launches.size() * KC_CHAIN_MAX_BATCH, nullptr);
    auto drop_outs = [&] {
        for (auto *o : outs) plane_release(o);
    };
    for (size_t li = 0; li < e->launches.size(); ++li) {
        const ReplayLaunch &L = e->launches[li];
        ChainProgram P = L.prog;
        kc_plane *src[KC_CHAIN_MAX_BATCH][KC_CHAIN_MAX_IN] = {};
        for (int b = 0; b < L.batch; ++b) {
            kc_plane *&o = outs[li * KC_CHAIN_MAX_BATCH + b];
            int s = plane_new_mem(L.w, L.h, &o);
            if (s != KC_OK) {
                drop_outs();
                return s;
            }
            P.out[b] = o->dptr;
            P.out_pitch[b] = (uint32_t)(o->pitch / 16);
            for (uint32_t k = 0; k < P.n_in; ++k)
                if (L.in_from[b][k] >= 0) {
                    const kc_plane *res = outs[(size_t)L.in_from[b][k] * KC_CHAIN_MAX_BATCH + L.in_ch[b][k]];
                    P.in[b][k] = res->dptr;
                    P.in_pitch[b][k] = (uint32_t)(res->pitch / 16);
                } else {
                    src[b][k] = L.in_plane[b][k];
                }
        }
        const uint64_t px4 = 4ull * L.w * L.h;
        P.nt_mask = chain_cache_policy(L.in_refs, P.n_in, px4 * L.batch, px4 * L.batch);
        uint64_t packed_saved = 0;
        hipError_t he = chain_dispatch(P, L.batch, L.mode, L.w, L.h, outs[li * KC_CHAIN_MAX_BATCH]->pitch, src, L.in_refs, &packed_saved);
        if (he == hipErrorNotReady) {
            drop_outs();
            return KC_OK;
        }
        if (he != hipSuccess) {
            drop_outs();
            return hip_fail(he, "launch_chain (replay)");
        }
        c.launches++;
        c.alg_bytes += (uint64_t)L.batch * px4 * (P.n_in + 1) - packed_saved;
    }
    c.counters["replayed_evaluations"]++;

    kc_plane *planes[4] = { nullptr, nullptr, nullptr, nullptr };
    std::vector<kc_plane *> consts;
    for (int p = 0; p < e->n_planes; ++p) {
        if (e->out_l[p] >= 0) planes[p] = outs[(size_t)e->out_l[p] * KC_CHAIN_MAX_BATCH + e->out_b[p]];
        else {
            planes[p] = plane_new_const(e->w, e->h, e->cval[p]);
            consts.push_back(planes[p]);
        }
    }
    kc_image *img = image_new(e->n_planes, planes);
    for (auto *q : consts) plane_release(q);
    drop_outs();

    for (uint32_t d : e->dropped) lg.remove_nodes_data(d);
    lg.slot_datas[id].push_back(SlotData{ id, e->root_slot, img });
    for (auto &ps : e->post_state) lg.node_state[ps.first] = ps.second;
    for (uint32_t ch : e->changed_ids) lg.changed.insert(ch);
    *hit = true;
    return KC_OK;
}

struct ReplayRecorder {
    kc_live_graph::ReplayEntry *entry = nullptr;
    ReplayCapture cap;
    uint64_t launches0 = 0;
    std::unordered_set<uint32_t> changed0;
    std::set<const void *> resident0;
    std::set<const kc_plane *> resident_planes;
};

static void note_resident(ReplayRecorder &r, const kc_image *img)
{
    for (int p = 0; p < img->n; ++p)
        if (img->planes[p]->kind == kc_plane::MEM) {
            r.resident0.insert(img->planes[p]->dptr);
            r.resident_planes.insert(img->planes[p]);
        }
}

ReplayRecorder *replay_begin(kc_live_graph &lg, uint32_t id)
{
    Context &c = ctx();
    if (lg.use_cache || lg.auto_update || !c.opt.fusion || !c.opt.replay || c.capture || lg.depth > 0) return nullptr;
    if (lg.g.nodes.size() > 4096) return nullptr;
    auto *r = new ReplayRecorder();
    auto *e = new kc_live_graph::ReplayEntry();
    r->entry = e;
    e->root = id;
    e->ghash = graph_content_hash(lg.g);
    e->pre_state.assign(lg.node_state.begin(), lg.node_state.end());
    for (auto &kv : lg.slot_datas)
        for (auto &sd : kv.second) {
            if (sd.node_id == id) continue;
            image_retain(sd.image);
            e->pre_slots.push_back({ sd.node_id, sd.slot_id, sd.image });
            note_resident(*r, sd.image);
        }
    for (auto &em : lg.embedded) {
        if (em.full_h != 0) {
            delete e;
            delete r;
            return nullptr;
        }
        image_retain(em.image);
        e->embedded.push_back(em);
        note_resident(*r, em.image);
    }
    r->launches0 = c.launches;
    r->changed0 = lg.changed;
    c.capture = &r->cap;
    return r;
}

void replay_end(kc_live_graph &lg, uint32_t id, ReplayRecorder *r, int s)
{
    if (!r) return;
    Context &c = ctx();
    c.capture = nullptr;
    std::unique_ptr<ReplayRecorder> own(r);
    std::unique_ptr<kc_live_graph::ReplayEntry> e(r->entry);
    lg.replay_clear();
    if (s != KC_OK || !r->cap.ok || r->cap.launches.empty() || c.launches - r->launches0 != r->cap.launches.size()) return;
    std::unordered_map<uint32_t, int> pre(e->pre_state.begin(), e->pre_state.end());
    if (pre.size() != lg.node_state.size()) return;
    {
        std::unordered_set<uint32_t> had;
        for (auto &h : e->pre_slots) had.insert(h.node);
        for (auto &n : lg.g.nodes)
            if (!had.count(n.node_id) && !recordable_type(n.type)) return;
    }
    for (auto &kv : lg.node_state) {
        auto it = pre.find(kv.first);
        if (it == pre.end()) return;
        if (it->second != kv.second) {
            const Node *n = lg.g.find(kv.first);
            if (!n || !recordable_type(n->type)) return;
            e->post_state.push_back({ kv.first, kv.second });
        }
    }
    std::unordered_map<uint64_t, kc_image *> before;
    for (auto &h : e->pre_slots) before[((uint64_t)h.node << 32) | h.slot] = h.img;
    std::unordered_set<uint32_t> has_after;
    const SlotData *root_sd = nullptr;
    size_t root_slots = 0;
    for (auto &kv : lg.slot_datas)
        for (auto &sd : kv.second) {
            has_after.insert(sd.node_id);
            if (sd.node_id == id) {
                root_sd = &sd;
                ++root_slots;
                continue;
            }
            auto it = before.find(((uint64_t)sd.node_id << 32) | sd.slot_id);
            if (it == before.end() || it->second != sd.image) return;
        }
    if (!root_sd || root_slots != 1) return;
    std::unordered_set<uint32_t> dropped;
    for (auto &h : e->pre_slots)
        if (!has_after.count(h.node)) dropped.insert(h.node);
    dropped.insert(id);
    for (auto &h : e->pre_slots)
        if (!dropped.count(h.node) && !lg.find_slot(h.node, h.slot)) return;
    e->dropped.assign(dropped.begin(), dropped.end());
    const kc_image *img = root_sd->image;
    ReplayCapture &cap = r->cap;
    e->w = img->w();
    e->h = img->h();
    e->root_slot = root_sd->slot_id;
    e->n_planes = img->n;
    for (int p = 0; p < img->n; ++p) {
        const kc_plane *pl = img->planes[p];
        e->out_l[p] = e->out_b[p] = -1;
        if (pl->kind == kc_plane::CONST) {
            e->cval[p] = pl->cval;
            continue;
        }
        for (size_t li = 0; li < cap.launches.size(); ++li)
            for (int b = 0; b < cap.launches[li].batch; ++b)
                if (cap.launches[li].planes[b] == pl && cap.launches[li].w == img->w() && cap.launches[li].h == img->h()) {
                    e->out_l[p] = (int)li;
                    e->out_b[p] = b;
                }
        if (e->out_l[p] < 0) return;
    }
    for (size_t li = 0; li < cap.launches.size(); ++li) {
        ReplayLaunch &L = cap.launches[li];
        for (int b = 0; b < L.batch; ++b)
            for (uint32_t k = 0; k < L.prog.n_in; ++k) {
                L.in_from[b][k] = L.in_ch[b][k] = -1;
                for (size_t lj = li; lj-- > 0 && L.in_from[b][k] < 0;)
                    for (int bj = 0; bj < cap.launches[lj].batch; ++bj)
                        if (cap.launches[lj].prog.out[bj] == L.prog.in[b][k]) {
                            if (cap.launches[lj].w != L.w || cap.launches[lj].h != L.h) return;
                            L.in_from[b][k] = (int)lj;
                            L.in_ch[b][k] = bj;
                        }
                if (L.in_from[b][k] < 0 && !r->resident0.count(L.prog.in[b][k])) return;
                if (L.in_from[b][k] >= 0 || !r->resident_planes.count(L.in_plane[b][k])) L.in_plane[b][k] = nullptr;
            }
    }
    for (uint32_t ch : lg.changed)
        if (!r->changed0.count(ch)) e->changed_ids.push_back(ch);
    e->launches = std::move(cap.launches);
    lg.replay = e.release();
}

}

void kc_live_graph::replay_clear()
{
    delete replay;
    replay = nullptr;
}
```

kanter_core_amd/csrc/specialize.cpp:

```cpp
#include <dlfcn.h>
#include <sys/stat.h>
#include <unistd.h>

#include <condition_variable>
#include <cstdio>
#include <cstdlib>
#include <cstring>
#include <thread>

#include "kc_runtime.hpp"

namespace kc {

extern const char kJitChainProgramH[];
extern const char kJitPowPositiveInc[];
extern const char kJitUpsampleH[];
extern const char kJitUpsampleChainInc[];
extern const char kJitChainPackH[] __attribute__((weak));

namespace {

typedef struct _hiprtcProgram *hiprtcProgram;
struct Rtc {
    void *lib = nullptr;
    int (*create)(hiprtcProgram *, const char *, const char *, int, const char **, const char **) = nullptr;
    int (*compile)(hiprtcProgram, int, const char **) = nullptr;
    int (*log_size)(hiprtcProgram, size_t *) = nullptr;
    int (*log)(hiprtcProgram, char *) = nullptr;
    int (*code_size)(hiprtcProgram, size_t *) = nullptr;
    int (*code)(hiprtcProgram, char *) = nullptr;
    int (*destroy)(hiprtcProgram *) = nullptr;
    int (*version)(int *, int *) = nullptr;
    bool ok = false;
    bool tried = false;
};

void specialize_stop_at_exit();

Rtc &rtc()
{
    static Rtc r;
    static std::once_flag once;
    std::call_once(once, [] {
        r.tried = true;
        for (const char *name : { "libhiprtc.so", "libhiprtc.so.7", "/opt/rocm/lib/libhiprtc.so" }) {
            r.lib = dlopen(name, RTLD_NOW | RTLD_LOCAL);
            if (r.lib) break;
        }
        if (!r.lib) return;
#define KC_RTC_SYM(field, sym) *(void **)(&r.field) = dlsym(r.lib, sym)
        KC_RTC_SYM(create, "hiprtcCreateProgram");
        KC_RTC_SYM(compile, "hiprtcCompileProgram");
        KC_RTC_SYM(log_size, "hiprtcGetProgramLogSize");
        KC_RTC_SYM(log, "hiprtcGetProgramLog");
        KC_RTC_SYM(code_size, "hiprtcGetCodeSize");
        KC_RTC_SYM(code, "hiprtcGetCode");
        KC_RTC_SYM(destroy, "hiprtcDestroyProgram");
        KC_RTC_SYM(version, "hiprtcVersion");
#undef KC_RTC_SYM
        r.ok = r.create && r.compile && r.log_size && r.log && r.code_size && r.code && r.destroy;
        if (r.ok) std::atexit(specialize_stop_at_exit);
    });
    return r;
}

struct Signature {
    uint32_t n_in = 0, n_ops = 0;
    int32_t start_src = 0;
    bool flat = false;
    uint32_t up_taps = 0;
    bool up_wide = false;
    uint32_t nt_mask = 0;
    uint32_t quads = 1;
    uint32_t in_tiers = 0;
    uint32_t word[KC_CHAIN_MAX_OPS] = {};

    std::string key() const
    {
        std::string k((const char *)&n_in, sizeof n_in);
        k.append((const char *)&n_ops, sizeof n_ops);
        k.append((const char *)&start_src, sizeof start_src);
        k.push_back(flat ? 'f' : 'p');
        k.push_back((char)('0' + up_taps));
        k.push_back(up_wide ? 'w' : 'n');
        k.append((const char *)&nt_mask, sizeof nt_mask);
        k.append((const char *)word, sizeof(uint32_t) * n_ops);
        if (quads > 1) {
            k.push_back('q');
            k.push_back((char)('0' + quads));
        }
        if (in_tiers) {
            k.push_back('t');
            k.append((const char *)&in_tiers, sizeof in_tiers);
        }
        return k;
    }
};

constexpr uint32_t kQuadsWarm = 2, kQuadsMaxOps = 16;
std::atomic<int> g_chain_quads{ 0 };

uint32_t chain_quads_for(const Signature &s, uint64_t total_units)
{
    if (s.up_taps || !s.flat || s.n_in < 1 || s.n_ops > kQuadsMaxOps || total_units > 0xF0000000ull) return 1;
    bool plain = false;
    for (uint32_t k = 0; k < s.n_in; ++k) plain |= !(s.nt_mask & KC_CHAIN_NT_BIT(k));
    if (!plain || !s.nt_mask) return 1;
    for (uint32_t i = 0; i < s.n_ops; ++i) {
        const uint32_t code = s.word[i] & 0xffu;
        if (code == CH_DIV_L || code == CH_DIV_R || code == CH_POW_L || code == CH_POW_R) return 1;
    }
    const int forced = g_chain_quads.load(std::memory_order_relaxed);
    return forced ? (uint32_t)forced : kQuadsWarm;
}

bool pack_program_ok(const ChainProgram &P)
{
    if (P.n_ops < 1 || P.n_ops > kQuadsMaxOps || P.n_in < 1 || P.rows != 1) return false;
    for (uint32_t i = 0; i < P.n_ops; ++i) {
        const uint32_t code = ((i & 1u) ? P.step[0][i / 2].b.word : P.step[0][i / 2].a.word) & 0xffu;
        if (code == CH_DIV_L || code == CH_DIV_R || code == CH_POW_L || code == CH_POW_R) return false;
    }
    return true;
}

Signature signature_of(const ChainProgram &P, const UpsampleArgs *U = nullptr)
{
    Signature s;
    s.n_in = P.n_in;
    s.n_ops = P.n_ops;
    s.start_src = P.start_src;
    s.flat = U ? false : P.rows == 1;
    {
        uint32_t valid = 0x100u;
        for (uint32_t k = 0; k < (U ? P.n_in - 1u : P.n_in); ++k) valid |= KC_CHAIN_NT_BIT(k);
        s.nt_mask = P.nt_mask & valid;
    }
    if (U) {
        s.up_taps = U->H.taps;
        s.up_wide = U->tile_w == 1024;
    }
    for (uint32_t i = 0; i < P.n_ops; ++i) s.word[i] = (i & 1u) ? P.step[0][i / 2].b.word : P.step[0][i / 2].a.word;
    if (!U && s.flat) s.in_tiers = P.n_in >= 16 ? P.in_tiers : P.in_tiers & ((1u << (2 * P.n_in)) - 1u);
    s.quads = chain_quads_for(s, (uint64_t)P.rows * P.row_units);
    return s;
}

static int spec_wg()
{
    static int wg = [] {
        int v = 256;
        if (const char *e = std::getenv("KC_SPEC_WG")) {
            const int x = std::atoi(e);
            if (x == 64 || x == 128 || x == 256 || x == 512 || x == 1024) v = x;
        }
        return v;
    }();
    return wg;
}

std::string kernel_name(const Signature &s)
{
    uint32_t h = 2166136261u;
    for (unsigned char c : s.key()) h = (h ^ c) * 16777619u;
    char buf[32];
    std::snprintf(buf, sizeof buf, s.up_taps ? "kc_upchain_%08x" : "kc_chain_%08x", h);
    return buf;
}

static const char kPackedF4[] = R"KCF4(typedef float raw4 __attribute__((ext_vector_type(4)));
typedef float f2 __attribute__((ext_vector_type(2)));
typedef unsigned long long __attribute__((may_alias)) rec64;
static __device__ __forceinline__ f2 pk_sub(f2 a, f2 b)
{
    f2 d;
    asm("v_pk_add_f32 %0, %1, %2 neg_lo:[0,1] neg_hi:[0,1]" : "=v"(d) : "v"(a), "v"(b));
    return d;
}
struct kconst {
    rec64 rec;  // { word, c }
    __device__ __forceinline__ operator float() const { return __builtin_bit_cast(float, (unsigned int)(rec >> 32)); }
    __device__ __forceinline__ f2 minus(f2 b) const
    {
        f2 d;
        asm("v_pk_add_f32 %0, %1, %2 op_sel_hi:[0,1] neg_lo:[0,1] neg_hi:[0,1]" : "=v"(d) : "s"(rec >> 32), "v"(b));
        return d;
    }
};
struct f4 {
    f2 lo, hi;
    f4() = default;
    __device__ __forceinline__ f4(float x, float y, float z, float w) : lo{ x, y }, hi{ z, w } {}
    __device__ __forceinline__ f4(f2 l, f2 h) : lo(l), hi(h) {}
    __device__ __forceinline__ f4(raw4 v) : lo(v.xy), hi(v.zw) {}
    __device__ __forceinline__ raw4 raw() const { return raw4{ lo.x, lo.y, hi.x, hi.y }; }
};
static __device__ __forceinline__ f4 operator+(f4 a, f4 b) { return f4(a.lo + b.lo, a.hi + b.hi); }
static __device__ __forceinline__ f4 operator*(f4 a, f4 b) { return f4(a.lo * b.lo, a.hi * b.hi); }
static __device__ __forceinline__ f4 operator-(f4 a, f4 b) { return f4(pk_sub(a.lo, b.lo), pk_sub(a.hi, b.hi)); }
static __device__ __forceinline__ f4 operator-(kconst c, f4 b) { return f4(c.minus(b.lo), c.minus(b.hi)); }
static __device__ __forceinline__ f4 operator/(f4 a, f4 b) { return f4(a.raw() / b.raw()); }
struct StepRecView { kconst c; };
struct StepPairView { StepRecView a, b; };
struct StepTableView {
    const ChainStepPair *p;
    __device__ __forceinline__ StepPairView operator[](unsigned int i) const
    {
        const rec64 *q = reinterpret_cast<const rec64 *>(p + i);
        return StepPairView{ { { q[0] } }, { { q[1] } } };
    }
};
)KCF4";

static std::string step_expr(const Signature &s, uint32_t i, const char *in_prefix, const char *in_suffix)
{
    const uint32_t code = s.word[i] & 0xffu, from = (s.word[i] >> 8) & 0xffu, level = (s.word[i] >> 16) & 3u;
    char c[48], x[96];
    std::snprintf(c, sizeof c, "pp[%u].%c.c", i / 2, (i & 1u) ? 'b' : 'a');
    if (from == 0)
        std::snprintf(x, sizeof x, "f4{ %s, %s, %s, %s }", c, c, c, c);
    else if (from == (uint32_t)KC_CHAIN_SRC_SAVED)
        std::snprintf(x, sizeof x, "saved%u", level);
    else
        std::snprintf(x, sizeof x, "%s%u%s", in_prefix, from - 1, in_suffix);
    switch (code) {
    case CH_SAVE_LOAD: return "(saved" + std::to_string(level) + " = acc, " + x + ")";
    case CH_ADD: return std::string("acc + ") + x;
    case CH_SUB_L: return std::string("acc - ") + x;
    case CH_SUB_R: return std::string(x) + " - acc";
    case CH_MUL: return std::string("acc * ") + x;
    case CH_DIV_L: return std::string("acc / ") + x;
    case CH_DIV_R: return std::string(x) + " / acc";
    case CH_POW_L: return std::string("pow4(acc, ") + x + ", pow_tab)";
    case CH_POW_R: return std::string("pow4(") + x + ", acc, pow_tab)";
    case CH_ADD_INV: return std::string(c) + " - (acc + " + x + ")";
    case CH_SUBL_INV: return std::string(c) + " - (acc - " + x + ")";
    case CH_SUBR_INV: return std::string(c) + " - (" + x + " - acc)";
    case CH_MUL_INV: return std::string(c) + " - (acc * " + x + ")";
    default: return std::string();
    }
}

static std::string generate_up(const Signature &s)
{
    std::string src;
    src.reserve(32768);
    src += "namespace kc {\n";
    src += kJitChainProgramH;
    src += kJitUpsampleH;
// ... 28 lines not shown
                  kernel_name(s).c_str(), s.n_in, s.up_taps, KC_UPSAMPLE_ROWS, s.up_wide ? "true" : "false", s.nt_mask);
    src += buf;
    return src;
}

static std::string load_expr(const Signature &s, uint32_t k, const std::string &at)
{
    const uint32_t tier = KC_CHAIN_TIER(s.in_tiers, k);
    const bool nt = (s.nt_mask & KC_CHAIN_NT_BIT(k)) != 0;
    const std::string in = "P.in[b][" + std::to_string(k) + "]";
    std::string ptr;
    if (tier == (uint32_t)KC_PACK_FIX24)
        ptr = "reinterpret_cast<const pack_u3a *>(reinterpret_cast<const char *>(" + in + ") + (unsigned long long)(" + at + ") * 12u)";
    else if (tier == (uint32_t)KC_PACK_U8)
        ptr = "&reinterpret_cast<const unsigned int *>(" + in + ")[" + at + "]";
    else
        ptr = "&reinterpret_cast<const raw4 *>(" + in + ")[" + at + "]";
    const std::string v = nt ? "__builtin_nontemporal_load(" + ptr + ")" : "*(" + ptr + ")";
    return tier == (uint32_t)KC_PACK_FIX24 ? "pack_decode_fix24(" + v + ")" : tier == (uint32_t)KC_PACK_U8 ? "pack_decode_u8(" + v + ")" : v;
}

static std::string generate_quads(const Signature &s, int SPEC_WG)
{
    std::string src;
    char buf[320];
    std::snprintf(buf, sizeof buf,
                  "    const unsigned int n = P.rows * P.row_units;\n"
                  "    const unsigned int idx = blockIdx.x * %uu + threadIdx.x;\n    if (idx >= n) return;\n",
                  s.quads * (uint32_t)SPEC_WG);
    src += buf;
    for (uint32_t u = 0; u < s.quads; ++u) {
        if (u == 0)
            src += "    const unsigned int at0 = idx;\n";
        else {
            std::snprintf(buf, sizeof buf, "    const unsigned int at%u = idx + %uu < n ? idx + %uu : n - 1u;\n", u, u * SPEC_WG, u * SPEC_WG);
            src += buf;
        }
        for (uint32_t k = 0; k < s.n_in; ++k) {
            if (KC_CHAIN_TIER(s.in_tiers, k)) {
                src += "    const f4 in" + std::to_string(k) + "_" + std::to_string(u) + " = " + load_expr(s, k, "at" + std::to_string(u)) + ";\n";
                continue;
            }
            if (s.nt_mask & KC_CHAIN_NT_BIT(k))
                std::snprintf(buf, sizeof buf, "    const f4 in%u_%u = __builtin_nontemporal_load(&reinterpret_cast<const raw4 *>(P.in[b][%u])[at%u]);\n", k, u, k, u);
            else
                std::snprintf(buf, sizeof buf, "    const f4 in%u_%u = reinterpret_cast<const raw4 *>(P.in[b][%u])[at%u];\n", k, u, k, u);
            src += buf;
        }
    }
    src += "    const StepTableView pp{ P.step[b] };\n";
    for (uint32_t u = 0; u < s.quads; ++u) {
        char suffix[8];
        std::snprintf(suffix, sizeof suffix, "_%u", u);
        std::snprintf(buf, sizeof buf, "    f4 out%u;\n    {\n", u);
        src += buf;
        if (s.start_src < 0)
            src += "        f4 acc = f4{ P.start_c[b], P.start_c[b], P.start_c[b], P.start_c[b] };\n";
        else {
            std::snprintf(buf, sizeof buf, "        f4 acc = in%d%s;\n", s.start_src, suffix);
            src += buf;
        }
        src += "        f4 saved0 = acc, saved1 = acc, saved2 = acc;\n";
        for (uint32_t i = 0; i < s.n_ops; ++i) {
            const std::string e = step_expr(s, i, "in", suffix);
            if (e.empty()) return std::string();
            src += "        acc = " + e + ";\n";
        }
        std::snprintf(buf, sizeof buf, "        out%u = acc;\n    }\n", u);
        src += buf;
    }
    for (uint32_t u = 0; u < s.quads; ++u) {
        std::snprintf(buf, sizeof buf, "    if (idx + %uu < n) ", u * SPEC_WG);
        src += u ? buf : "    ";
        std::snprintf(buf, sizeof buf,
                      s.nt_mask & 0x100u ? "__builtin_nontemporal_store(out%u.raw(), &reinterpret_cast<raw4 *>(P.out[b])[idx + %uu]);\n"
                                         : "reinterpret_cast<raw4 *>(P.out[b])[idx + %uu] = out%u.raw();\n",
                      s.nt_mask & 0x100u ? u : u * SPEC_WG, s.nt_mask & 0x100u ? u * SPEC_WG : u);
        src += buf;
    }
    src += "}\n";
    return src;
}

std::string generate(const Signature &s)
{
    if (s.up_taps) return generate_up(s);
    const int SPEC_WG = spec_wg();
    bool pow = false;
    for (uint32_t i = 0; i < s.n_ops; ++i) pow |= (s.word[i] & 0xffu) == CH_POW_L || (s.word[i] & 0xffu) == CH_POW_R;
    std::string src;
    src.reserve(16384);
    src += "namespace kc {\n";
    src += kJitChainProgramH;
    src += kPackedF4;
    if (s.in_tiers) {
        const char *pack_text = kJitChainPackH;
        if (!pack_text) return std::string();
        src += pack_text;
    }
    if (pow) {
        src += kJitPowPositiveInc;
        src += "static __device__ __noinline__ float pow_general(float a, float b) { return (float)pow((double)a, (double)b); }\n"
               "static __device__ __forceinline__ float kc_powf(float a, float b, const PowCtx &pw)\n"
               "{\n"
               "    if (a > 0.0f && a < __builtin_inff() && __builtin_fabsf(b) < __builtin_inff()) return pow_positive(a, b, pw);\n"
               "    return pow_general(a, b);\n"
               "}\n"
               "static __device__ __forceinline__ f4 pow4(f4 a, f4 b, const PowCtx &t) { return f4{ kc_powf(a.lo.x, b.lo.x, t), kc_powf(a.lo.y, b.lo.y, t), kc_powf(a.hi.x, b.hi.x, t), kc_powf(a.hi.y, b.hi.y, t) }; }\n";
    }
    src += "}  // namespace kc\nusing namespace kc;\n";
    char buf[256];
    std::snprintf(buf, sizeof buf, "extern \"C\" __global__ __launch_bounds__(%d) void %s(const ChainProgram P)\n{\n", SPEC_WG,
                  kernel_name(s).c_str());
    src += buf;
    if (pow) src += "    __shared__ double pow_lds[KC_POW_TABLE_DOUBLES];\n    const PowCtx pow_tab = pow_setup(pow_lds);\n";
    src += "    const unsigned int b = blockIdx.y;\n";
    if (s.quads > 1) {
        const std::string body = generate_quads(s, SPEC_WG);
        return body.empty() ? body : src + body;
    }
    std::snprintf(buf, sizeof buf, "    const unsigned int idx = blockIdx.x * %du + threadIdx.x;\n", SPEC_WG);
    src += buf;
    src += "    if (idx >= P.rows * P.row_units) return;\n";
    if (s.flat)
        src += "    const unsigned int row = 0u, col = idx;\n";
    else
        src += "    const unsigned int row = idx / P.row_units, col = idx - row * P.row_units;\n";
    for (uint32_t k = 0; k < s.n_in; ++k) {
        if (KC_CHAIN_TIER(s.in_tiers, k)) {
            src += "    const f4 in" + std::to_string(k) + " = " + load_expr(s, k, "col") + ";\n";
            continue;
        }
        if (s.nt_mask & KC_CHAIN_NT_BIT(k))
            std::snprintf(buf, sizeof buf, "    const f4 in%u = __builtin_nontemporal_load(&reinterpret_cast<const raw4 *>(P.in[b][%u])[row * P.in_pitch[b][%u] + col]);\n", k, k, k);
        else
            std::snprintf(buf, sizeof buf, "    const f4 in%u = reinterpret_cast<const raw4 *>(P.in[b][%u])[row * P.in_pitch[b][%u] + col];\n", k, k, k);
        src += buf;
    }
    src += "    const StepTableView pp{ P.step[b] };\n";
    if (s.start_src < 0)
        src += "    f4 acc = f4{ P.start_c[b], P.start_c[b], P.start_c[b], P.start_c[b] };\n";
    else {
        std::snprintf(buf, sizeof buf, "    f4 acc = in%d;\n", s.start_src);
        src += buf;
    }
    src += "    f4 saved0 = acc, saved1 = acc, saved2 = acc;\n";
    for (uint32_t i = 0; i < s.n_ops; ++i) {
        const std::string e = step_expr(s, i, "in", "");
        if (e.empty()) return std::string();
        src += "    acc = " + e + ";\n";
    }
    if (s.nt_mask & 0x100u)
        src += "    __builtin_nontemporal_store(acc.raw(), &reinterpret_cast<raw4 *>(P.out[b])[row * P.out_pitch[b] + col]);\n}\n";
    else
        src += "    reinterpret_cast<raw4 *>(P.out[b])[row * P.out_pitch[b] + col] = acc.raw();\n}\n";
    return src;
}

static const char *const kCompileOpts[] = { "--gpu-architecture=gfx950", "-O3", "-ffp-contract=off", "-fno-fast-math",
                                            "-fhip-fp32-correctly-rounded-divide-sqrt" };
constexpr int kNumCompileOpts = (int)(sizeof kCompileOpts / sizeof *kCompileOpts);

uint64_t fnv64(const void *data, size_t n, uint64_t h = 1469598103934665603ull)
{
    const unsigned char *p = (const unsigned char *)data;
    for (size_t i = 0; i < n; ++i) h = (h ^ p[i]) * 1099511628211ull;
    return h;
}

// ... 198 lines not shown
    return true;
}

struct Entry {
    enum State { COUNTING, QUEUED, READY, FAILED } state = COUNTING;
    uint32_t sightings = 0;
    Signature sig;
    hipModule_t module = nullptr;
    hipFunction_t fn = nullptr;
};

struct Spec {
    std::mutex mu;
    std::condition_variable cv, idle_cv;
    std::map<std::string, Entry> cache;
    std::unordered_map<uint64_t, std::pair<std::string, Entry *>> by_hash;
    std::deque<std::string> queue;
    std::thread worker;
    bool worker_running = false, stopping = false;
    int busy = 0;
    std::atomic<int> mode{ 1 };
    uint32_t after = 2;
    int device = -1;
    uint64_t compiled = 0, failed = 0, launches = 0, loaded_from_disk = 0;
    std::string last_log;

    void stop()
    {
        {
            std::lock_guard<std::mutex> lk(mu);
            stopping = true;
            for (auto &key : queue) {
                auto it = cache.find(key);
                if (it != cache.end() && it->second.state == Entry::QUEUED) {
                    it->second.state = Entry::COUNTING;
                    it->second.sightings = 0;
                }
            }
            queue.clear();
        }
        cv.notify_all();
        idle_cv.notify_all();
        if (worker.joinable()) worker.join();
        std::lock_guard<std::mutex> lk(mu);
        worker_running = false;
        stopping = false;
    }
};

Spec &spec()
{
    static Spec *s = new Spec();
    return *s;
}

void specialize_stop_at_exit() { spec().stop(); }

bool compile_entry(const Signature &sig, hipModule_t *module, hipFunction_t *fn, std::string *log, bool disk_only = false)
{
    const std::string src = generate(sig);
    if (src.empty()) {
        *log = "unknown step code";
        return false;
    }
    std::vector<char> code;
    if (disk_load(sig, src, code)) {
        if (load_code(sig, code, module, fn, log)) return true;
        std::lock_guard<std::mutex> lk(disk().mu);
        disk().hits--;
        disk().rejected++;
    }
    if (disk_only) {
        *log = "not in the kernel cache";
        return false;
    }
    if (!rtc_compile(src, code, log)) return false;
    if (!load_code(sig, code, module, fn, log)) return false;
    disk_store(sig, src, code);
    if (const char *m = std::getenv("KC_KERNEL_CACHE_MANIFEST")) {
        if (FILE *f = std::fopen(m, "a")) {
            std::fprintf(f, "{\"name\": \"%s\", \"n_in\": %u, \"start_src\": %d, \"flat\": %d, \"nt_mask\": %u, \"up_taps\": %u, \"up_wide\": %d, \"words\": [",
                         kernel_name(sig).c_str(), sig.n_in, sig.start_src, sig.flat ? 1 : 0, sig.nt_mask, sig.up_taps, sig.up_wide ? 1 : 0);
            for (uint32_t k = 0; k < sig.n_ops; ++k) std::fprintf(f, "%s%u", k ? ", " : "", sig.word[k]);
            if (sig.in_tiers) std::fprintf(f, "], \"in_tiers\": %u}\n", sig.in_tiers);
            else std::fprintf(f, "]}\n");
            std::fclose(f);
        }
    }
    return true;
}

void finish(Spec &S, const std::string &key, bool ok, hipModule_t m, hipFunction_t f, const std::string &log, bool from_disk = false)
{
    auto it = S.cache.find(key);
    if (it == S.cache.end()) {
        if (ok) (void)hipModuleUnload(m);
        return;
    }
    if (ok) {
        it->second.module = m;
        it->second.fn = f;
        it->second.state = Entry::READY;
        if (from_disk) S.loaded_from_disk++;
        else S.compiled++;
    } else {
        it->second.state = Entry::FAILED;
        S.failed++;
        S.last_log = log;
    }
}

void worker_main()
{
    Spec &S = spec();
    if (S.device >= 0) (void)hipSetDevice(S.device);
    std::unique_lock<std::mutex> lk(S.mu);
    for (;;) {
        S.cv.wait(lk, [&] { return S.stopping || !S.queue.empty(); });
        if (S.stopping) return;
        const std::string key = S.queue.front();
        S.queue.pop_front();
        auto it = S.cache.find(key);
        if (it == S.cache.end()) continue;
        const Signature sig = it->second.sig;
        S.busy++;
        lk.unlock();
        hipModule_t m = nullptr;
        hipFunction_t f = nullptr;
        std::string log;
        const uint64_t hits0 = disk_hits();
        const bool ok = compile_entry(sig, &m, &f, &log);
        const bool from_disk = ok && disk_hits() != hits0;
        lk.lock();
        S.busy--;
        finish(S, key, ok, m, f, log, from_disk);
        S.idle_cv.notify_all();
    }
}

}

static uint64_t signature_hash(const Signature &s)
{
    uint64_t h = 1469598103934665603ull;
    auto mix = [&](uint64_t v) { h = (h ^ v) * 1099511628211ull; };
    mix(s.n_in);
    mix(s.n_ops);
    mix((uint64_t)(int64_t)s.start_src);
    mix(s.flat ? 1 : 0);
    mix(s.up_taps);
    mix(s.up_wide ? 1 : 0);
    mix(s.nt_mask);
    mix(s.quads);
    mix(s.in_tiers);
    for (uint32_t i = 0; i < s.n_ops; ++i) mix(s.word[i]);
    return h;
}

static bool same_signature(const Signature &a, const Signature &b)
{
    return a.n_in == b.n_in && a.n_ops == b.n_ops && a.start_src == b.start_src && a.flat == b.flat && a.up_taps == b.up_taps &&
           a.up_wide == b.up_wide && a.nt_mask == b.nt_mask && a.quads == b.quads && a.in_tiers == b.in_tiers &&
           std::memcmp(a.word, b.word, sizeof(uint32_t) * a.n_ops) == 0;
}

static hipFunction_t spec_lookup(const Signature &sig)
{
    Spec &S = spec();
    if (S.mode.load(std::memory_order_relaxed) == 0) return nullptr;
    const uint64_t h = signature_hash(sig);
    {
        std::lock_guard<std::mutex> fast(S.mu);
        auto it = S.by_hash.find(h);
        if (it != S.by_hash.end() && it->second.second->state == Entry::READY && same_signature(it->second.second->sig, sig))
            return it->second.second->fn;
    }
    const std::string key = sig.key();
    std::unique_lock<std::mutex> lk(S.mu);
    if (S.mode == 2) {
        auto it = S.cache.find(key);
        if (it != S.cache.end() && it->second.state == Entry::QUEUED)
            S.idle_cv.wait(lk, [&] { return S.cache[key].state != Entry::QUEUED || !S.worker_running; });
    }
    Entry &e = S.cache[key];
    if (e.state == Entry::READY) {
        e.sig = sig;
        S.by_hash[h] = { key, &e };
        return e.fn;
    }
    if (e.state != Entry::COUNTING) return nullptr;
    e.sightings++;
    if (e.sightings == 1 && S.mode == 1) {
        hipModule_t m = nullptr;
        hipFunction_t f = nullptr;
        std::string log;
        e.sig = sig;
        if (compile_entry(sig, &m, &f, &log, true)) {
            e.module = m;
            e.fn = f;
            e.state = Entry::READY;
            S.loaded_from_disk++;
            S.by_hash[h] = { key, &e };
            return f;
        }
    }
    if (S.mode == 1 && e.sightings < S.after) return nullptr;
    e.sig = sig;
    if (S.mode == 2) {
        e.state = Entry::QUEUED;
        lk.unlock();
        hipModule_t m = nullptr;
        hipFunction_t f = nullptr;
        std::string log;
        const uint64_t hits0 = disk_hits();
        const bool ok = compile_entry(sig, &m, &f, &log);
        const bool from_disk = ok && disk_hits() != hits0;
        lk.lock();
        finish(S, key, ok, m, f, log, from_disk);
        return ok ? f : nullptr;
    }
    e.state = Entry::QUEUED;
    S.queue.push_back(key);
    if (!S.worker_running) {
        S.device = ctx().device;
        S.stopping = false;
        S.worker = std::thread(worker_main);
        S.worker_running = true;
    }
    lk.unlock();
    S.cv.notify_one();
    return nullptr;
}

hipError_t launch_chain_specialized(const ChainProgram &P, int batch, hipStream_t s, bool *launched, uint32_t *nt_mask, uint32_t *quads)
{
    *launched = false;
    if (P.n_ops < 1 || P.n_ops > (uint32_t)KC_CHAIN_MAX_OPS || P.n_in > (uint32_t)KC_CHAIN_MAX_IN) return hipSuccess;
    const uint64_t total = (uint64_t)P.rows * P.row_units;
    if (total == 0 || total > 0xFFFFFFFFull) return hipSuccess;
    const Signature sig = signature_of(P);
    hipFunction_t fn = spec_lookup(sig);
    if (!fn) return hipSuccess;
    size_t size = sizeof(ChainProgram);
    const int SPEC_WG = spec_wg();
    void *extra[] = { HIP_LAUNCH_PARAM_BUFFER_POINTER, (void *)&P, HIP_LAUNCH_PARAM_BUFFER_SIZE, &size, HIP_LAUNCH_PARAM_END };
    const uint64_t per_block = (uint64_t)SPEC_WG * sig.quads;
    const unsigned gx = (unsigned)((total + per_block - 1) / per_block);
    hipError_t e = hipModuleLaunchKernel(fn, gx, (unsigned)batch, 1, SPEC_WG, 1, 1, 0, s, nullptr, extra);
    if (e == hipSuccess) {
        *launched = true;
        if (nt_mask) *nt_mask = sig.nt_mask;
        if (quads) *quads = sig.quads;
        std::lock_guard<std::mutex> lk(spec().mu);
        spec().launches++;
    }
    return e;
}

bool chain_pack_program_ok(const ChainProgram &P) { return pack_program_ok(P); }

hipError_t launch_upsample_chain_specialized(const ChainProgram &P, int batch, const UpsampleArgs &U, hipStream_t s, bool *launched)
{
    *launched = false;
    if (P.n_ops < 1 || P.n_ops > (uint32_t)KC_CHAIN_MAX_OPS || P.n_in < 1 || P.n_in > (uint32_t)KC_CHAIN_INTERP_IN) return hipSuccess;
    if (!upsample_args_ok(U, batch) || (U.H.taps != 1 && U.H.taps != 3)) return hipSuccess;
    if (U.H.ratio == 2) return hipSuccess;
    hipFunction_t fn = spec_lookup(signature_of(P, &U));
    if (!fn) return hipSuccess;
    struct alignas(16) Params {
        ChainProgram P;
        UpsampleArgs U;
    };
    static_assert(sizeof(ChainProgram) % alignof(UpsampleArgs) == 0, "the second kernel argument follows the first without padding");
    static thread_local Params params;
    params.P = P;
    params.U = U;
    size_t size = sizeof(Params);
    void *extra[] = { HIP_LAUNCH_PARAM_BUFFER_POINTER, (void *)&params, HIP_LAUNCH_PARAM_BUFFER_SIZE, &size, HIP_LAUNCH_PARAM_END };
    const dim3 grid = upsample_grid(U, batch);
    hipError_t e = hipModuleLaunchKernel(fn, grid.x, grid.y, grid.z, 256, 1, 1, (unsigned)upsample_lds_bytes(U), s, nullptr, extra);
    if (e == hipSuccess) {
        *launched = true;
        std::lock_guard<std::mutex> lk(spec().mu);
        spec().launches++;
    }
    return e;
}

int specialize_set_mode(int mode, int after)
{
    Spec &S = spec();
    if (mode < 0 || mode > 2) return KC_ERR_INVALID_ARG;
    {
        std::lock_guard<std::mutex> lk(S.mu);
        S.mode.store(mode);
        if (after >= 1) S.after = (uint32_t)after;
    }
    if (mode == 0) S.stop();
    return KC_OK;
}

int specialize_get_mode()
{
    Spec &S = spec();
    return S.mode.load();
}

void specialize_wait()
{
    Spec &S = spec();
    std::unique_lock<std::mutex> lk(S.mu);
    S.idle_cv.wait(lk, [&] { return S.stopping || (S.queue.empty() && S.busy == 0); });
}

void specialize_stats(uint64_t *compiled, uint64_t *failed, uint64_t *launches, uint64_t *pending)
{
    Spec &S = spec();
    std::lock_guard<std::mutex> lk(S.mu);
    if (compiled) *compiled = S.compiled;
    if (failed) *failed = S.failed;
    if (launches) *launches = S.launches;
    if (pending) *pending = S.queue.size() + (uint64_t)S.busy;
}

std::string specialize_last_log()
{
    Spec &S = spec();
    std::lock_guard<std::mutex> lk(S.mu);
    return S.last_log;
}

void specialize_shutdown()
{
    Spec &S = spec();
    S.stop();
    std::lock_guard<std::mutex> lk(S.mu);
    for (auto &kv : S.cache)
        if (kv.second.module) (void)hipModuleUnload(kv.second.module);
    S.by_hash.clear();
    S.cache.clear();
}

int specialize_set_chain_quads(int quads)
{
    if (quads != 0 && quads != 1 && quads != 2 && quads != 4) return KC_ERR_INVALID_ARG;
    g_chain_quads.store(quads);
    return KC_OK;
}

int specialize_get_chain_quads() { return g_chain_quads.load(); }

std::string specialize_source(const ChainProgram &P, const UpsampleArgs *U) { return generate(signature_of(P, U)); }

int specialize_compile_only(const ChainProgram &P, std::string *log, const UpsampleArgs *U)
{
    if (!rtc().ok) {
        *log = "libhiprtc not available";
        return KC_ERR_UNSUPPORTED;
    }
    const std::string src = generate(signature_of(P, U));
    if (src.empty()) return KC_ERR_GENERIC;
    std::vector<char> code;
    return rtc_compile(src, code, log) ? KC_OK : KC_ERR_GENERIC;
}

int kernel_cache_set_dir(const char *dir)
{
    DiskCache &d = disk();
    std::lock_guard<std::mutex> lk(d.mu);
    resolve_dirs_locked(d, dir && *dir ? dir : nullptr);
    return KC_OK;
}

void kernel_cache_stats(uint64_t *hits, uint64_t *rejected, uint64_t *written, uint64_t *kernels_loaded)
{
    {
        DiskCache &d = disk();
        std::lock_guard<std::mutex> lk(d.mu);
        if (hits) *hits = d.hits;
        if (rejected) *rejected = d.rejected;
        if (written) *written = d.written;
    }
    Spec &S = spec();
    std::lock_guard<std::mutex> lk(S.mu);
    if (kernels_loaded) *kernels_loaded = S.loaded_from_disk;
}

bool kernel_cache_populated()
{
    DiskCache &d = disk();
    std::vector<std::string> dirs;
    {
        std::lock_guard<std::mutex> lk(d.mu);
        if (!d.resolved) resolve_dirs_locked(d, nullptr);
        dirs = d.read_dirs;
        if (dirs.empty()) return false;
        if (d.hits) return true;
    }
    static std::map<std::string, bool> seen;
    for (auto &dir : dirs) {
        auto it = seen.find(dir);
        if (it == seen.end()) {
            bool any = false;
            std::string probe = dir + "/.populated";
            any = access(probe.c_str(), R_OK) == 0;
            it = seen.emplace(dir, any).first;
        }
        if (it->second) return true;
    }
    return false;
}

int kernel_cache_precompile(const uint32_t *words, uint32_t n_ops, uint32_t n_in, int32_t start_src, bool flat, uint32_t nt_mask, uint32_t in_tiers,
                            uint32_t up_taps, bool up_wide, const char *dir, std::string *log)
{
    if (in_tiers && (!flat || up_taps || (n_in < 16 && in_tiers >> (2 * n_in)))) return KC_ERR_INVALID_ARG;
    for (uint32_t k = 0; k < n_in; ++k)
        if (KC_CHAIN_TIER(in_tiers, k) == 3u) return KC_ERR_INVALID_ARG;
    if (!words || n_ops < 1 || n_ops > (uint32_t)KC_CHAIN_MAX_OPS || n_in > (uint32_t)KC_CHAIN_MAX_IN || !dir || !*dir) return KC_ERR_INVALID_ARG;
    Signature sig;
    sig.n_in = n_in;
    sig.n_ops = n_ops;
    sig.start_src = start_src;
    sig.flat = flat;
    sig.nt_mask = nt_mask;
    sig.up_taps = up_taps;
    sig.up_wide = up_wide;
    sig.in_tiers = in_tiers;
    for (uint32_t i = 0; i < n_ops; ++i) sig.word[i] = words[i];
    sig.quads = chain_quads_for(sig, 0);
    const std::string src = generate(sig);
    if (src.empty()) {
        *log = "unknown step code";
        return KC_ERR_INVALID_ARG;
    }
    std::vector<char> code;
    if (!rtc_compile(src, code, log)) return rtc().ok ? KC_ERR_GENERIC : KC_ERR_UNSUPPORTED;
    if (!make_dirs(dir) || !disk_store_in(dir, sig, src, code)) {
        *log = std::string("cannot write into ") + dir;
        return KC_ERR_IO;
    }
    if (FILE *f = std::fopen((std::string(dir) + "/.populated").c_str(), "w")) std::fclose(f);
    return KC_OK;
}

}
```

Before: 7.132 million.

## Fuse replayed chain launches into tapped kernels that store intermediate outputs

Adds a tapped chain kernel that runs a short per-pixel op chain once and writes every needed intermediate result (taps) to its output plane. Replay groups consecutive chain launches into one such launch, avoiding separate kernel launches and the re-read of intermediate planes from memory. The feature is on by default and needs runtime-compiled kernels. It adds replay-plan complexity and falls back to the old path when pitches or program shapes don't fit.

```diff
diff --git a/bindings/rust/kanter_core_amd_sys.rs b/bindings/rust/kanter_core_amd_sys.rs
--- a/bindings/rust/kanter_core_amd_sys.rs
+++ b/bindings/rust/kanter_core_amd_sys.rs
@@ -322,6 +322,10 @@
     pub fn kc_kernel_cache_precompile(words: *const u32, n_ops: u32, n_in: u32, start_src: i32, flat: i32, nt_mask: u32, up_taps: u32, up_wide: i32, dir: *const c_char) -> i32;
     pub fn kc_specialize_reset() -> i32;
     pub fn kc_kernel_cache_precompile_packed(words: *const u32, n_ops: u32, n_in: u32, start_src: i32, flat: i32, nt_mask: u32, in_tiers: u32, dir: *const c_char) -> i32;
+    pub fn kc_set_replay_taps(on: i32) -> i32;
+    pub fn kc_get_replay_taps() -> i32;
+    pub fn kc_specialize_compile_check_taps(words: *const u32, n_ops: u32, n_in: u32, start_src: i32, nt_mask: u32, tap_mask: u32, source: *mut c_char, cap: usize) -> i32;
+    pub fn kc_kernel_cache_precompile_taps(words: *const u32, n_ops: u32, n_in: u32, start_src: i32, nt_mask: u32, tap_mask: u32, dir: *const c_char) -> i32;
     pub fn kc_set_pack_sources(mode: i32) -> i32;
     pub fn kc_get_pack_sources() -> i32;
     pub fn kc_set_pack_budget_mb(mb: i32) -> i32;
diff --git a/include/kanter_core_amd.h b/include/kanter_core_amd.h
--- a/include/kanter_core_amd.h
+++ b/include/kanter_core_amd.h
@@ -118,6 +118,12 @@
 KC_API int kc_specialize_reset(void);
 KC_API int kc_kernel_cache_precompile_packed(const uint32_t *words, uint32_t n_ops, uint32_t n_in, int start_src, int flat,
                                              uint32_t nt_mask, uint32_t in_tiers, const char *dir);
+KC_API int kc_set_replay_taps(int on);
+KC_API int kc_get_replay_taps(void);
+KC_API int kc_specialize_compile_check_taps(const uint32_t *words, uint32_t n_ops, uint32_t n_in, int start_src, uint32_t nt_mask,
+                                            uint32_t tap_mask, char *source, size_t cap);
+KC_API int kc_kernel_cache_precompile_taps(const uint32_t *words, uint32_t n_ops, uint32_t n_in, int start_src, uint32_t nt_mask,
+                                           uint32_t tap_mask, const char *dir);
 KC_API int kc_set_pack_sources(int mode);
 KC_API int kc_get_pack_sources(void);
 KC_API int kc_set_pack_budget_mb(int mb);
diff --git a/kanter_core_amd/__init__.py b/kanter_core_amd/__init__.py
--- a/kanter_core_amd/__init__.py
+++ b/kanter_core_amd/__init__.py
@@ -4,7 +4,7 @@
                   init, is_initialized, mix_process, resize_image, separate_rgba_process, set_fusion, set_stream,
                   shutdown, stats, sync, value_process, set_specialize, get_specialize, specialize_wait,
                   specialize_stats, specialize_compile_check, Partition, PartitionPolicy, NodeKind, set_resize_mode,
-                  get_resize_mode, resize_upsample_plan, resize_down2_plan, stats_counter, specialize_compile_check_upsample, specialize_compile_check_mask, set_chain_quads, get_chain_quads, set_pack_sources, get_pack_sources, set_pack_budget_mb, get_pack_budget_mb, set_cache_policy, get_cache_policy, set_option, get_option, comm_unique_id, comm_init,
+                  get_resize_mode, resize_upsample_plan, resize_down2_plan, stats_counter, specialize_compile_check_upsample, specialize_compile_check_mask, set_chain_quads, get_chain_quads, set_replay_taps, get_replay_taps, specialize_compile_check_taps, set_pack_sources, get_pack_sources, set_pack_budget_mb, get_pack_budget_mb, set_cache_policy, get_cache_policy, set_option, get_option, comm_unique_id, comm_init,
                   comm_destroy, comm_info, comm_stats, comm_transport, comm_gather_bands, PlanKind, pool_trim, kernel_cache_set_dir, kernel_cache_stats,
                   kernel_cache_precompile, specialize_reset, U8Pipe, device_image_desc, DEVICE_SRGB, DEVICE_GRAY,
                   ChannelStats, STATS_HISTOGRAM, STATS_SRGB, BC_SRGB, BC6H, BC7, BC_BLOCK_BYTES, BC_PUNCH_THROUGH, bc_punch_through_ref, bc1_punch_through_block,
diff --git a/kanter_core_amd/_abi.py b/kanter_core_amd/_abi.py
--- a/kanter_core_amd/_abi.py
+++ b/kanter_core_amd/_abi.py
@@ -340,6 +340,10 @@
     "kc_kernel_cache_precompile": (C.c_int, [C.POINTER(C.c_uint32), C.c_uint32, C.c_uint32, C.c_int, C.c_int, C.c_uint32, C.c_uint32, C.c_int, C.c_char_p]),
     "kc_specialize_reset": (C.c_int, []),
     "kc_kernel_cache_precompile_packed": (C.c_int, [C.POINTER(C.c_uint32), C.c_uint32, C.c_uint32, C.c_int, C.c_int, C.c_uint32, C.c_uint32, C.c_char_p]),
+    "kc_set_replay_taps": (C.c_int, [C.c_int]),
+    "kc_get_replay_taps": (C.c_int, []),
+    "kc_specialize_compile_check_taps": (C.c_int, [C.POINTER(C.c_uint32), C.c_uint32, C.c_uint32, C.c_int, C.c_uint32, C.c_uint32, C.c_char_p, C.c_size_t]),
+    "kc_kernel_cache_precompile_taps": (C.c_int, [C.POINTER(C.c_uint32), C.c_uint32, C.c_uint32, C.c_int, C.c_uint32, C.c_uint32, C.c_char_p]),
     "kc_set_pack_sources": (C.c_int, [C.c_int]),
     "kc_get_pack_sources": (C.c_int, []),
     "kc_set_pack_budget_mb": (C.c_int, [C.c_int]),
diff --git a/kanter_core_amd/api.py b/kanter_core_amd/api.py
--- a/kanter_core_amd/api.py
+++ b/kanter_core_amd/api.py
@@ -212,6 +212,22 @@
 
 def get_chain_quads():
     return _lib.load().kc_get_chain_quads()
+
+
+def set_replay_taps(on):
+    _check(_lib.load().kc_set_replay_taps(int(on)))
+
+
+def get_replay_taps():
+    return _lib.load().kc_get_replay_taps()
+
+
+def specialize_compile_check_taps(words, n_in, tap_mask, nt_mask=0, start_src=0):
+    arr = (C.c_uint32 * len(words))(*words)
+    buf = C.create_string_buffer(1 << 17)
+    _check(_lib.load().kc_specialize_compile_check_taps(arr, len(words), int(n_in), int(start_src), int(nt_mask), int(tap_mask),
+                                                        buf, len(buf)))
+    return buf.value.decode()
 
 
 def set_pack_sources(mode):
diff --git a/kanter_core_amd/build.py b/kanter_core_amd/build.py
--- a/kanter_core_amd/build.py
+++ b/kanter_core_amd/build.py
@@ -8,14 +8,14 @@
 OBJ = os.path.join(HERE, "csrc", "build")
 LIB = os.path.join(HERE, "libkanter_core_amd.so")
 SOURCES = ["chain.hip", "upsample.hip", "resize_tile.hip", "resize_down.hip", "h2n.hip", "u8.hip", "chain1.hip", "down2.hip", "runtime.cpp",
-           "ops.cpp", "resize.cpp", "graph.cpp", "json.cpp", "png.cpp", "specialize.cpp", "partition.cpp", "bands.cpp", "comm.cpp", "replay.cpp",
+           "ops.cpp", "resize.cpp", "graph.cpp", "json.cpp", "png.cpp", "specialize.cpp", "partition.cpp", "bands.cpp", "comm.cpp", "replay.cpp", "replay_plan.cpp",
            "u8pipe.cpp", "devimage.hip", "devimage.cpp", "stats.hip", "stats.cpp", "bc.hip", "bc1a.hip", "bc7.hip", "bc6h.hip", "bc.cpp", "mip.hip", "mip_normals.hip", "mip_roughness.hip", "mip_alpha.hip", "mip_coverage.hip", "mip.cpp", "mip_export.cpp", "preview.hip", "preview.cpp", "sdf.hip", "sdf.cpp", "bc_decode.hip",
            "bc_decode.cpp", "bc_modes.hip", "chain_pack.hip", "chain_pack.cpp",
            "c_api.cpp"]
-HEADERS = ["kc_internal.hpp", "kc_runtime.hpp", "chain_program.h", "chain_pack.h", "preview_walk.h", "mip_steps.h", os.path.join("..", "..", "include", "kanter_core_amd.h"), "pow_positive.inc",
+HEADERS = ["kc_internal.hpp", "kc_runtime.hpp", "chain_program.h", "chain_taps.h", "replay_plan.h", "chain_pack.h", "preview_walk.h", "mip_steps.h", os.path.join("..", "..", "include", "kanter_core_amd.h"), "pow_positive.inc",
            "srgb_thresholds.inc", "streaming.h", "bc_blocks.h", "bc_modes.h", "upsample.h", "upsample_chain.inc", "chain_apply.inc", "chain_interp.inc", "resample.inc"]
 JIT_TEXTS = [("kJitChainProgramH", "chain_program.h"), ("kJitPowPositiveInc", "pow_positive.inc"), ("kJitUpsampleH", "upsample.h"),
-             ("kJitUpsampleChainInc", "upsample_chain.inc"), ("kJitChainPackH", "chain_pack.h")]
+             ("kJitUpsampleChainInc", "upsample_chain.inc"), ("kJitChainPackH", "chain_pack.h"), ("kJitChainTapsH", "chain_taps.h")]
 
 FLAGS = ["--offload-arch=gfx950", "-O3", "-std=c++17", "-fPIC", "-fvisibility=hidden", "-fno-fast-math",
          "-ffp-contract=off", "-fhip-fp32-correctly-rounded-divide-sqrt", "-Wall", "-Wno-unused-result"]
@@ -131,11 +131,16 @@
     L.kc_kernel_cache_precompile_packed.argtypes = [C.POINTER(C.c_uint32), C.c_uint32, C.c_uint32, C.c_int, C.c_int, C.c_uint32, C.c_uint32,
                                                     C.c_char_p]
     L.kc_kernel_cache_precompile_packed.restype = C.c_int
+    L.kc_kernel_cache_precompile_taps.argtypes = [C.POINTER(C.c_uint32), C.c_uint32, C.c_uint32, C.c_int, C.c_uint32, C.c_uint32, C.c_char_p]
+    L.kc_kernel_cache_precompile_taps.restype = C.c_int
     L.kc_last_error.restype = C.c_char_p
 
     def one(e):
         words = (C.c_uint32 * len(e["words"]))(*e["words"])
-        if e.get("in_tiers"):
+        if e.get("taps"):
+            rc = L.kc_kernel_cache_precompile_taps(words, len(e["words"]), e["n_in"], e["start_src"], e["nt_mask"], e["taps"],
+                                                   KERNEL_CACHE.encode())
+        elif e.get("in_tiers"):
             rc = L.kc_kernel_cache_precompile_packed(words, len(e["words"]), e["n_in"], e["start_src"], e["flat"], e["nt_mask"],
                                                      e["in_tiers"], KERNEL_CACHE.encode())
         else:
diff --git a/kanter_core_amd/csrc/c_api.cpp b/kanter_core_amd/csrc/c_api.cpp
--- a/kanter_core_amd/csrc/c_api.cpp
+++ b/kanter_core_amd/csrc/c_api.cpp
@@ -453,6 +453,68 @@
 }
 KC_CATCH
 
+int kc_set_replay_taps(int on)
+try {
+    Lock lk(ctx().mu);
+    const int s = replay_set_taps(on);
+    if (s != KC_OK) set_error("kc_set_replay_taps accepts 0 or 1");
+    return s;
+}
+KC_CATCH
+
+int kc_get_replay_taps(void)
+try {
+    return replay_get_taps();
+}
+catch (...) {
+    return 0;
+}
+
+static bool tapped_program_from_words(ChainProgram &P, const uint32_t *words, uint32_t n_ops, uint32_t n_in, int start_src, uint32_t nt_mask)
+{
+    if (!words || n_ops < 1 || n_ops > (uint32_t)KC_TAP_MAX_OPS || n_in > (uint32_t)KC_CHAIN_MAX_IN || start_src < -1 || start_src >= (int)n_in)
+        return false;
+    std::memset(&P, 0, sizeof P);
+    P.n_ops = n_ops;
+    P.n_in = n_in;
+    P.start_src = start_src;
+    P.rows = 1;
+    P.row_units = 1;
+    P.nt_mask = nt_mask;
+    for (uint32_t i = 0; i < n_ops; ++i) {
+        if ((words[i] & 0xffu) > CH_MUL_INV || ((words[i] >> 8) & 0xffu) > n_in || words[i] >> 16) return false;
+        ((i & 1u) ? P.step[0][i / 2].b : P.step[0][i / 2].a).word = words[i];
+    }
+    return true;
+}
+
+int kc_specialize_compile_check_taps(const uint32_t *words, uint32_t n_ops, uint32_t n_in, int start_src, uint32_t nt_mask,
+                                     uint32_t tap_mask, char *source, size_t cap)
+try {
+    ChainProgram P;
+    KC_ARG(tapped_program_from_words(P, words, n_ops, n_in, start_src, nt_mask));
+    if (source && cap) {
+        const std::string src = specialize_source_tapped(P, tap_mask);
+        std::snprintf(source, cap, "%s", src.c_str());
+    }
+    std::string log;
+    int s = specialize_compile_only_tapped(P, tap_mask, &log);
+    if (s != KC_OK) set_error("tapped chain kernel did not compile: " + log);
+    return s;
+}
+KC_CATCH
+
+int kc_kernel_cache_precompile_taps(const uint32_t *words, uint32_t n_ops, uint32_t n_in, int start_src, uint32_t nt_mask,
+                                    uint32_t tap_mask, const char *dir)
+try {
+    KC_ARG(words && dir && tap_mask && n_ops >= 1 && n_ops <= (uint32_t)KC_TAP_MAX_OPS);
+    std::string log = "tap_mask: one bit per record, the last record's set";
+    const int s = kernel_cache_precompile(words, n_ops, n_in, start_src, true, nt_mask, 0, 0, false, dir, &log, tap_mask);
+    if (s != KC_OK) set_error("kernel cache: " + log);
+    return s;
+}
+KC_CATCH
+
 int kc_set_pack_sources(int mode)
 try {
     Lock lk(ctx().mu);
diff --git a/kanter_core_amd/csrc/chain_taps.h b/kanter_core_amd/csrc/chain_taps.h
--- /dev/null
+++ b/kanter_core_amd/csrc/chain_taps.h
@@ -0,0 +1,18 @@
+enum { KC_TAP_MAX_OPS = 16, KC_TAP_MAX = KC_TAP_MAX_OPS };
+
+struct TapProgram {
+    unsigned int n_ops;
+    unsigned int n_in;
+    unsigned int row_units;
+    unsigned int rows;
+    int start_src;
+    unsigned int nt_mask;
+    unsigned int in_tiers;
+    unsigned int tap_mask;
+    const float *in[KC_CHAIN_MAX_BATCH][KC_CHAIN_MAX_IN];
+    float start_c[KC_CHAIN_MAX_BATCH];
+    float *tap[KC_CHAIN_MAX_BATCH][KC_TAP_MAX];
+    ChainStepPair step[KC_CHAIN_MAX_BATCH][KC_TAP_MAX_OPS / 2];
+};
+static_assert(sizeof(TapProgram) <= 4096, "a launch passes at most 4 KB of kernel arguments: lower KC_TAP_MAX");
+static_assert(KC_TAP_MAX <= KC_TAP_MAX_OPS && KC_TAP_MAX_OPS <= 32, "one tap per record at most, and tap_mask is one word");
diff --git a/kanter_core_amd/csrc/kc_internal.hpp b/kanter_core_amd/csrc/kc_internal.hpp
--- a/kanter_core_amd/csrc/kc_internal.hpp
+++ b/kanter_core_amd/csrc/kc_internal.hpp
@@ -16,6 +16,7 @@
 namespace kc {
 
 #include "chain_program.h"
+#include "chain_taps.h"
 #include "upsample.h"
 
 struct Options {
diff --git a/kanter_core_amd/csrc/kc_runtime.hpp b/kanter_core_amd/csrc/kc_runtime.hpp
--- a/kanter_core_amd/csrc/kc_runtime.hpp
+++ b/kanter_core_amd/csrc/kc_runtime.hpp
@@ -452,7 +452,12 @@
 void kernel_cache_stats(uint64_t *hits, uint64_t *rejected, uint64_t *written, uint64_t *kernels_loaded);
 bool kernel_cache_populated();
 int kernel_cache_precompile(const uint32_t *words, uint32_t n_ops, uint32_t n_in, int32_t start_src, bool flat, uint32_t nt_mask, uint32_t in_tiers,
-                            uint32_t up_taps, bool up_wide, const char *dir, std::string *log);
+                            uint32_t up_taps, bool up_wide, const char *dir, std::string *log, uint32_t tap_mask = 0);
+hipError_t launch_chain_tapped(const ChainProgram &P, int batch, uint32_t tap_mask, float *const (*taps)[KC_TAP_MAX], hipStream_t s, bool *launched);
+std::string specialize_source_tapped(const ChainProgram &P, uint32_t tap_mask);
+int specialize_compile_only_tapped(const ChainProgram &P, uint32_t tap_mask, std::string *log);
+int replay_set_taps(int on);
+int replay_get_taps();
 
 int u8_pipe_create(uint32_t w, uint32_t h, int channels, int depth, kc_u8_pipe **out);
 int u8_pipe_free(kc_u8_pipe *p);
diff --git a/kanter_core_amd/csrc/replay.cpp b/kanter_core_amd/csrc/replay.cpp
--- a/kanter_core_amd/csrc/replay.cpp
+++ b/kanter_core_amd/csrc/replay.cpp
@@ -1,8 +1,28 @@
 #include "kc_runtime.hpp"
+#include "replay_plan.h"
 
 using namespace kc;
 
+static_assert((int)KC_PLAN_MAX_IN == (int)KC_CHAIN_MAX_IN && (int)KC_PLAN_MAX_BATCH == (int)KC_CHAIN_MAX_BATCH && (int)KC_PLAN_MAX_OPS == (int)KC_TAP_MAX_OPS,
+              "replay_plan.h repeats these constants to stay free of the library's headers");
+
 struct kc_live_graph::ReplayEntry {
+    bool use_cache = false;
+    struct NodeOut {
+        uint32_t node = 0, slot = 0, w = 0, h = 0;
+        int n_planes = 0;
+        int out_l[4] = { -1, -1, -1, -1 };
+        int out_b[4] = { -1, -1, -1, -1 };
+        float cval[4] = { 0, 0, 0, 0 };
+    };
+    std::vector<NodeOut> node_outs;
+    std::unordered_set<uint32_t> replaced;
+    struct TapGroup {
+        PlanGroup plan;
+        ChainProgram prog;
+        uint32_t in_refs[KC_CHAIN_MAX_IN] = {};
+    };
+    std::vector<TapGroup> groups;
     uint32_t root = 0;
     uint64_t ghash = 0;
     std::vector<std::pair<uint32_t, int>> pre_state;
@@ -16,12 +36,6 @@
     std::vector<uint32_t> dropped;
     std::vector<uint32_t> changed_ids;
     std::vector<ReplayLaunch> launches;
-    uint32_t w = 0, h = 0;
-    uint32_t root_slot = 0;
-    int n_planes = 0;
-    int out_l[4] = { -1, -1, -1, -1 };
-    int out_b[4] = { -1, -1, -1, -1 };
-    float cval[4] = { 0, 0, 0, 0 };
 
     ~ReplayEntry()
     {
@@ -65,25 +79,79 @@
            t == KC_NODE_OUTPUT_GRAY || t == KC_NODE_OUTPUT_RGBA || t == KC_NODE_EMBED;
 }
 
-static size_t slot_count_except(const kc_live_graph &lg, uint32_t node)
+static size_t slot_count_except(const kc_live_graph &lg, const std::unordered_set<uint32_t> &nodes)
 {
     size_t n = 0;
     for (auto &kv : lg.slot_datas)
-        if (kv.first != node) n += kv.second.size();
+        if (!nodes.count(kv.first)) n += kv.second.size();
     return n;
+}
+
+static std::atomic<int> g_replay_taps{ 1 };
+
+int replay_set_taps(int on)
+{
+    if (on != 0 && on != 1) return KC_ERR_INVALID_ARG;
+    g_replay_taps.store(on);
+    return KC_OK;
+}
+
+int replay_get_taps() { return g_replay_taps.load(); }
+
+static hipError_t replay_launch_group(const kc_live_graph::ReplayEntry &e, const kc_live_graph::ReplayEntry::TapGroup &G,
+                                      const std::vector<kc_plane *> &outs, bool *launched)
+{
+    *launched = false;
+    Context &c = ctx();
+    const PlanGroup &g = G.plan;
+    const ReplayLaunch &F = e.launches[g.first];
+    const uint32_t row_units = (F.w + 3) / 4;
+    ChainProgram P = G.prog;
+    P.rows = 1;
+    P.row_units = row_units * F.h;
+    float *taps[KC_CHAIN_MAX_BATCH][KC_TAP_MAX] = {};
+    for (uint32_t t = 0; t < g.count; ++t)
+        for (int b = 0; b < F.batch; ++b) {
+            const kc_plane *o = outs[(size_t)(g.first + t) * KC_CHAIN_MAX_BATCH + b];
+            if (o->pitch != (size_t)row_units * 16) return hipSuccess;
+            taps[b][t] = o->dptr;
+        }
+    for (uint32_t s = 0; s < g.n_in; ++s) {
+        const ReplayLaunch &L = e.launches[g.in[s].launch];
+        const uint32_t k = g.in[s].k;
+        for (int b = 0; b < F.batch; ++b) {
+            if (L.in_from[b][k] >= 0) {
+                const kc_plane *res = outs[(size_t)L.in_from[b][k] * KC_CHAIN_MAX_BATCH + L.in_ch[b][k]];
+                if (res->pitch != (size_t)row_units * 16) return hipSuccess;
+                P.in[b][s] = res->dptr;
+            } else {
+                P.in[b][s] = L.prog.in[b][k];
+            }
+            P.in_pitch[b][s] = row_units;
+        }
+    }
+    const uint64_t px4 = 4ull * F.w * F.h;
+    P.nt_mask = chain_cache_policy(G.in_refs, P.n_in, px4 * F.batch, px4 * F.batch * g.count);
+    hipError_t he = launch_chain_tapped(P, F.batch, g.tap_mask, taps, c.stream, launched);
+    if (he != hipSuccess || !*launched) return he;
+    c.launches++;
+    c.alg_bytes += (uint64_t)F.batch * px4 * (P.n_in + g.count);
+    c.counters["tapped_launches"]++;
+    c.counters["tapped_nodes"] += g.count;
+    return hipSuccess;
 }
 
 int replay_try(kc_live_graph &lg, uint32_t id, bool *hit)
 {
     *hit = false;
     const kc_live_graph::ReplayEntry *e = lg.replay;
-    if (!e || e->root != id || lg.use_cache || lg.auto_update || !options().fusion || !options().replay) return KC_OK;
+    if (!e || e->root != id || lg.use_cache != e->use_cache || lg.auto_update || !options().fusion || !options().replay) return KC_OK;
     if (e->pre_state.size() != lg.node_state.size()) return KC_OK;
     for (auto &ps : e->pre_state) {
         auto it = lg.node_state.find(ps.first);
         if (it == lg.node_state.end() || it->second != ps.second) return KC_OK;
     }
-    if (slot_count_except(lg, id) != e->pre_slots.size()) return KC_OK;
+    if (slot_count_except(lg, e->replaced) != e->pre_slots.size()) return KC_OK;
     for (auto &h : e->pre_slots) {
         const SlotData *sd = lg.find_slot(h.node, h.slot);
         if (!sd || sd->image != h.img) return KC_OK;
@@ -101,17 +169,48 @@
     auto drop_outs = [&] {
         for (auto *o : outs) plane_release(o);
     };
+    auto new_outs = [&](size_t li) -> int {
+        const ReplayLaunch &L = e->launches[li];
+        for (int b = 0; b < L.batch; ++b) {
+            kc_plane *&o = outs[li * KC_CHAIN_MAX_BATCH + b];
+            if (!o) KC_TRY(plane_new_mem(L.w, L.h, &o));
+        }
+        return KC_OK;
+    };
+    size_t gi = e->groups.empty() || !g_replay_taps.load(std::memory_order_relaxed) ? e->groups.size() : 0;
     for (size_t li = 0; li < e->launches.size(); ++li) {
+        if (gi < e->groups.size() && e->groups[gi].plan.first == li) {
+            const PlanGroup &g = e->groups[gi].plan;
+            int s = KC_OK;
+            for (uint32_t t = 0; t < g.count && s == KC_OK; ++t) s = new_outs(li + t);
+            if (s != KC_OK) {
+                drop_outs();
+                return s;
+            }
+            bool launched = false;
+            hipError_t he = replay_launch_group(*e, e->groups[gi], outs, &launched);
+            ++gi;
+            if (he != hipSuccess) {
+                drop_outs();
+                return hip_fail(he, "launch_chain_tapped (replay)");
+            }
+            if (launched) {
+                li += g.count - 1;
+                continue;
+            }
+        }
         const ReplayLaunch &L = e->launches[li];
         ChainProgram P = L.prog;
         kc_plane *src[KC_CHAIN_MAX_BATCH][KC_CHAIN_MAX_IN] = {};
-        for (int b = 0; b < L.batch; ++b) {
-            kc_plane *&o = outs[li * KC_CHAIN_MAX_BATCH + b];
-            int s = plane_new_mem(L.w, L.h, &o);
+        {
+            const int s = new_outs(li);
             if (s != KC_OK) {
                 drop_outs();
                 return s;
             }
+        }
+        for (int b = 0; b < L.batch; ++b) {
+            kc_plane *o = outs[li * KC_CHAIN_MAX_BATCH + b];
             P.out[b] = o->dptr;
             P.out_pitch[b] = (uint32_t)(o->pitch / 16);
             for (uint32_t k = 0; k < P.n_in; ++k)
@@ -140,25 +239,78 @@
     }
     c.counters["replayed_evaluations"]++;
 
-    kc_plane *planes[4] = { nullptr, nullptr, nullptr, nullptr };
-    std::vector<kc_plane *> consts;
-    for (int p = 0; p < e->n_planes; ++p) {
-        if (e->out_l[p] >= 0) planes[p] = outs[(size_t)e->out_l[p] * KC_CHAIN_MAX_BATCH + e->out_b[p]];
-        else {
-            planes[p] = plane_new_const(e->w, e->h, e->cval[p]);
-            consts.push_back(planes[p]);
-        }
-    }
-    kc_image *img = image_new(e->n_planes, planes);
-    for (auto *q : consts) plane_release(q);
+    std::vector<kc_image *> imgs;
+    for (auto &no : e->node_outs) {
+        kc_plane *planes[4] = { nullptr, nullptr, nullptr, nullptr };
+        std::vector<kc_plane *> consts;
+        for (int p = 0; p < no.n_planes; ++p) {
+            if (no.out_l[p] >= 0) planes[p] = outs[(size_t)no.out_l[p] * KC_CHAIN_MAX_BATCH + no.out_b[p]];
+            else {
+                planes[p] = plane_new_const(no.w, no.h, no.cval[p]);
+                consts.push_back(planes[p]);
+            }
+        }
+        imgs.push_back(image_new(no.n_planes, planes));
+        for (auto *q : consts) plane_release(q);
+    }
     drop_outs();
 
     for (uint32_t d : e->dropped) lg.remove_nodes_data(d);
-    lg.slot_datas[id].push_back(SlotData{ id, e->root_slot, img });
+    for (size_t i = 0; i < e->node_outs.size(); ++i)
+        lg.slot_datas[e->node_outs[i].node].push_back(SlotData{ e->node_outs[i].node, e->node_outs[i].slot, imgs[i] });
     for (auto &ps : e->post_state) lg.node_state[ps.first] = ps.second;
     for (uint32_t ch : e->changed_ids) lg.changed.insert(ch);
     *hit = true;
     return KC_OK;
+}
+
+static void plan_groups(kc_live_graph::ReplayEntry &e)
+{
+    std::vector<PlanLaunch> pl(e.launches.size());
+    for (size_t li = 0; li < e.launches.size(); ++li) {
+        const ReplayLaunch &L = e.launches[li];
+        PlanLaunch &q = pl[li];
+        q.w = L.w;
+        q.h = L.h;
+        q.batch = L.batch;
+        q.flat_dense = L.prog.rows == 1 && L.w % 4 == 0;
+        q.start_src = L.prog.start_src;
+        q.n_in = L.prog.n_in;
+        for (uint32_t i = 0; i < L.prog.n_ops; ++i) {
+            q.words.push_back((i & 1u) ? L.prog.step[0][i / 2].b.word : L.prog.step[0][i / 2].a.word);
+            for (int b = 1; b < L.batch; ++b)
+                if (((i & 1u) ? L.prog.step[b][i / 2].b.word : L.prog.step[b][i / 2].a.word) != q.words.back()) q.flat_dense = false;
+        }
+        for (int b = 0; b < L.batch; ++b)
+            for (uint32_t k = 0; k < L.prog.n_in; ++k) {
+                q.in_from[b][k] = L.in_from[b][k];
+                q.in_ch[b][k] = L.in_ch[b][k];
+                q.in_ptr[b][k] = L.prog.in[b][k];
+            }
+    }
+    for (const PlanGroup &g : replay_plan_taps(pl, KC_TAP_MAX)) {
+        e.groups.emplace_back();
+        kc_live_graph::ReplayEntry::TapGroup &G = e.groups.back();
+        G.plan = g;
+        ChainProgram &P = G.prog;
+        std::memset(&P, 0, sizeof P);
+        const ReplayLaunch &F = e.launches[g.first];
+        P.n_ops = g.n_ops;
+        P.n_in = g.n_in;
+        P.start_src = g.start_src;
+        for (int b = 0; b < F.batch; ++b) P.start_c[b] = F.prog.start_c[b];
+        for (uint32_t i = 0; i < g.n_ops; ++i) {
+            const ReplayLaunch &L = e.launches[g.rec[i].launch];
+            const uint32_t j = g.rec[i].index;
+            for (int b = 0; b < F.batch; ++b) {
+                const ChainStepRec &from = (j & 1u) ? L.prog.step[b][j / 2].b : L.prog.step[b][j / 2].a;
+                ChainStepRec &to = (i & 1u) ? P.step[b][i / 2].b : P.step[b][i / 2].a;
+                to.word = g.word[i];
+                to.c = g.rec[i].c_from_start ? L.prog.start_c[b] : from.c;
+            }
+        }
+        for (uint32_t s = 0; s < g.n_in; ++s) G.in_refs[s] = e.launches[g.in[s].launch].in_refs[g.in[s].k];
+    }
 }
 
 struct ReplayRecorder {
@@ -182,17 +334,18 @@
 ReplayRecorder *replay_begin(kc_live_graph &lg, uint32_t id)
 {
     Context &c = ctx();
-    if (lg.use_cache || lg.auto_update || !c.opt.fusion || !c.opt.replay || c.capture || lg.depth > 0) return nullptr;
+    if (lg.auto_update || !c.opt.fusion || !c.opt.replay || c.capture || lg.depth > 0) return nullptr;
     if (lg.g.nodes.size() > 4096) return nullptr;
     auto *r = new ReplayRecorder();
     auto *e = new kc_live_graph::ReplayEntry();
     r->entry = e;
+    e->use_cache = lg.use_cache;
     e->root = id;
     e->ghash = graph_content_hash(lg.g);
     e->pre_state.assign(lg.node_state.begin(), lg.node_state.end());
     for (auto &kv : lg.slot_datas)
         for (auto &sd : kv.second) {
-            if (sd.node_id == id) continue;
+            if (sd.node_id == id && !lg.use_cache) continue;
             image_retain(sd.image);
             e->pre_slots.push_back({ sd.node_id, sd.slot_id, sd.image });
             note_resident(*r, sd.image);
@@ -239,50 +392,84 @@
             e->post_state.push_back({ kv.first, kv.second });
         }
     }
+    const bool cache = e->use_cache;
+    if (cache)
+        for (auto &ps : e->post_state) {
+            const Node *n = lg.g.find(ps.first);
+            if (!n || n->type != KC_NODE_MIX) return;
+        }
     std::unordered_map<uint64_t, kc_image *> before;
     for (auto &h : e->pre_slots) before[((uint64_t)h.node << 32) | h.slot] = h.img;
-    std::unordered_set<uint32_t> has_after;
-    const SlotData *root_sd = nullptr;
+    std::unordered_set<uint32_t> has_after, kept;
+    std::vector<const SlotData *> fresh;
     size_t root_slots = 0;
     for (auto &kv : lg.slot_datas)
         for (auto &sd : kv.second) {
             has_after.insert(sd.node_id);
-            if (sd.node_id == id) {
-                root_sd = &sd;
-                ++root_slots;
+            auto it = before.find(((uint64_t)sd.node_id << 32) | sd.slot_id);
+            if (it != before.end() && it->second == sd.image) {
+                kept.insert(sd.node_id);
                 continue;
             }
-            auto it = before.find(((uint64_t)sd.node_id << 32) | sd.slot_id);
-            if (it == before.end() || it->second != sd.image) return;
-        }
-    if (!root_sd || root_slots != 1) return;
-    std::unordered_set<uint32_t> dropped;
+            if (sd.node_id == id) ++root_slots;
+            else if (!cache) return;
+            fresh.push_back(&sd);
+        }
+    if (root_slots < 1 || (!cache && root_slots != 1)) return;
+    for (auto *sd : fresh) {
+        const Node *n = lg.g.find(sd->node_id);
+        if (kept.count(sd->node_id) || (cache && (!n || n->type != KC_NODE_MIX))) return;
+        e->replaced.insert(sd->node_id);
+    }
+    e->replaced.insert(id);
+    std::set<const void *> stale;
+    if (cache) {
+        std::vector<kc_live_graph::ReplayEntry::Held> keep;
+        for (auto &h : e->pre_slots) {
+            if (!e->replaced.count(h.node)) {
+                keep.push_back(h);
+                continue;
+            }
+            for (int p = 0; p < h.img->n; ++p)
+                if (h.img->planes[p]->kind == kc_plane::MEM) stale.insert(h.img->planes[p]->dptr);
+            image_release(h.img);
+        }
+        e->pre_slots.swap(keep);
+        for (auto &h : e->pre_slots)
+            for (int p = 0; p < h.img->n; ++p) stale.erase(h.img->planes[p]->kind == kc_plane::MEM ? h.img->planes[p]->dptr : nullptr);
+        for (auto &em : e->embedded)
+            for (int p = 0; p < em.image->n; ++p) stale.erase(em.image->planes[p]->kind == kc_plane::MEM ? em.image->planes[p]->dptr : nullptr);
+    }
+    std::unordered_set<uint32_t> dropped(e->replaced.begin(), e->replaced.end());
     for (auto &h : e->pre_slots)
         if (!has_after.count(h.node)) dropped.insert(h.node);
-    dropped.insert(id);
     for (auto &h : e->pre_slots)
         if (!dropped.count(h.node) && !lg.find_slot(h.node, h.slot)) return;
     e->dropped.assign(dropped.begin(), dropped.end());
-    const kc_image *img = root_sd->image;
     ReplayCapture &cap = r->cap;
-    e->w = img->w();
-    e->h = img->h();
-    e->root_slot = root_sd->slot_id;
-    e->n_planes = img->n;
-    for (int p = 0; p < img->n; ++p) {
-        const kc_plane *pl = img->planes[p];
-        e->out_l[p] = e->out_b[p] = -1;
-        if (pl->kind == kc_plane::CONST) {
-            e->cval[p] = pl->cval;
-            continue;
-        }
-        for (size_t li = 0; li < cap.launches.size(); ++li)
-            for (int b = 0; b < cap.launches[li].batch; ++b)
-                if (cap.launches[li].planes[b] == pl && cap.launches[li].w == img->w() && cap.launches[li].h == img->h()) {
-                    e->out_l[p] = (int)li;
-                    e->out_b[p] = b;
-                }
-        if (e->out_l[p] < 0) return;
+    for (auto *sd : fresh) {
+        const kc_image *img = sd->image;
+        kc_live_graph::ReplayEntry::NodeOut no;
+        no.node = sd->node_id;
+        no.slot = sd->slot_id;
+        no.w = img->w();
+        no.h = img->h();
+        no.n_planes = img->n;
+        for (int p = 0; p < img->n; ++p) {
+            const kc_plane *pl = img->planes[p];
+            if (pl->kind == kc_plane::CONST) {
+                no.cval[p] = pl->cval;
+                continue;
+            }
+            for (size_t li = 0; li < cap.launches.size(); ++li)
+                for (int b = 0; b < cap.launches[li].batch; ++b)
+                    if (cap.launches[li].planes[b] == pl && cap.launches[li].w == img->w() && cap.launches[li].h == img->h()) {
+                        no.out_l[p] = (int)li;
+                        no.out_b[p] = b;
+                    }
+            if (no.out_l[p] < 0) return;
+        }
+        e->node_outs.push_back(no);
     }
     for (size_t li = 0; li < cap.launches.size(); ++li) {
         ReplayLaunch &L = cap.launches[li];
@@ -296,13 +483,14 @@
                             L.in_from[b][k] = (int)lj;
                             L.in_ch[b][k] = bj;
                         }
-                if (L.in_from[b][k] < 0 && !r->resident0.count(L.prog.in[b][k])) return;
+                if (L.in_from[b][k] < 0 && (!r->resident0.count(L.prog.in[b][k]) || stale.count(L.prog.in[b][k]))) return;
                 if (L.in_from[b][k] >= 0 || !r->resident_planes.count(L.in_plane[b][k])) L.in_plane[b][k] = nullptr;
             }
     }
     for (uint32_t ch : lg.changed)
         if (!r->changed0.count(ch)) e->changed_ids.push_back(ch);
     e->launches = std::move(cap.launches);
+    if (cache) plan_groups(*e);
     lg.replay = e.release();
 }
 
diff --git a/kanter_core_amd/csrc/replay_plan.cpp b/kanter_core_amd/csrc/replay_plan.cpp
--- /dev/null
+++ b/kanter_core_amd/csrc/replay_plan.cpp
@@ -0,0 +1,122 @@
+#include "replay_plan.h"
+
+namespace kc {
+
+namespace {
+
+bool code_ok(uint32_t code) { return code <= 3u || (code >= 10u && code <= 13u); }
+
+bool eligible(const PlanLaunch &L)
+{
+    if (!L.flat_dense || L.batch < 1 || L.batch > KC_PLAN_MAX_BATCH || L.w == 0 || L.h == 0) return false;
+    if (L.words.empty() || L.words.size() > (size_t)KC_PLAN_MAX_OPS || L.n_in > (uint32_t)KC_PLAN_MAX_IN) return false;
+    if (L.start_src >= (int)L.n_in) return false;
+    for (uint32_t wd : L.words) {
+        const uint32_t from = (wd >> 8) & 0xffu;
+        if (!code_ok(wd & 0xffu) || from > L.n_in || (wd >> 16) != 0) return false;
+    }
+    return true;
+}
+
+bool same_input(const PlanLaunch &A, uint32_t ka, const PlanLaunch &B, uint32_t kb, int batch)
+{
+    for (int b = 0; b < batch; ++b) {
+        if (A.in_from[b][ka] != B.in_from[b][kb]) return false;
+        if (A.in_from[b][ka] >= 0 ? A.in_ch[b][ka] != B.in_ch[b][kb] : A.in_ptr[b][ka] != B.in_ptr[b][kb]) return false;
+    }
+    return true;
+}
+
+int run_input(PlanGroup &g, const std::vector<PlanLaunch> &all, uint32_t li, uint32_t k)
+{
+    const PlanLaunch &L = all[li];
+    for (int b = 0; b < L.batch; ++b)
+        if (L.in_from[b][k] >= (int)g.first) return -1;
+    for (uint32_t s = 0; s < g.n_in; ++s)
+        if (same_input(all[g.in[s].launch], g.in[s].k, L, k, L.batch)) return (int)s;
+    if (g.n_in >= (uint32_t)KC_PLAN_MAX_IN) return -1;
+    g.in[g.n_in] = { li, k };
+    return (int)g.n_in++;
+}
+
+bool append(PlanGroup &g, const std::vector<PlanLaunch> &all, uint32_t li, uint32_t max_taps)
+{
+    const PlanLaunch &L = all[li];
+    PlanGroup t = g;
+    bool swap = false;
+    if (t.count == 0) {
+        t.first = li;
+        t.start_src = -1;
+        if (L.start_src >= 0) {
+            t.start_src = run_input(t, all, li, (uint32_t)L.start_src);
+            if (t.start_src < 0) return false;
+        }
+    } else {
+        const PlanLaunch &F = all[t.first];
+        if (L.w != F.w || L.h != F.h || L.batch != F.batch || t.count >= max_taps) return false;
+        auto continues = [&](int k) {
+            for (int b = 0; b < L.batch; ++b)
+                if (L.in_from[b][k] != (int)li - 1 || L.in_ch[b][k] != b) return false;
+            return true;
+        };
+        if (L.start_src < 0 || !continues(L.start_src)) {
+            const uint32_t code = L.words[0] & 0xffu, from = (L.words[0] >> 8) & 0xffu;
+            if (code > 3u || from == 0 || (int)from - 1 == L.start_src || !continues((int)from - 1)) return false;
+            swap = true;
+        }
+    }
+    if (t.n_ops + L.words.size() > (size_t)KC_PLAN_MAX_OPS) return false;
+    for (uint32_t i = 0; i < L.words.size(); ++i) {
+        uint32_t wd = L.words[i];
+        const uint32_t from = (wd >> 8) & 0xffu;
+        t.rec[t.n_ops] = { li, i, false };
+        if (i == 0 && swap) {
+            const uint32_t code = wd & 0xffu;
+            wd = code == 1u ? 2u : code == 2u ? 1u : code;
+            if (L.start_src < 0) {
+                t.rec[t.n_ops].c_from_start = true;
+            } else {
+                const int s = run_input(t, all, li, (uint32_t)L.start_src);
+                if (s < 0) return false;
+                wd |= (uint32_t)(s + 1) << 8;
+            }
+        } else if (from) {
+            const int s = run_input(t, all, li, from - 1);
+            if (s < 0) return false;
+            wd = (wd & ~0xff00u) | ((uint32_t)(s + 1) << 8);
+        }
+        t.word[t.n_ops] = wd;
+        ++t.n_ops;
+    }
+    t.tap_mask |= 1u << (t.n_ops - 1);
+    ++t.count;
+    g = t;
+    return true;
+}
+
+}
+
+std::vector<PlanGroup> replay_plan_taps(const std::vector<PlanLaunch> &launches, uint32_t max_taps)
+{
+    std::vector<PlanGroup> groups;
+    if (max_taps > (uint32_t)KC_PLAN_MAX_OPS) max_taps = KC_PLAN_MAX_OPS;
+    if (max_taps < 2) return groups;
+    PlanGroup g;
+    auto close = [&] {
+        if (g.count >= 2) groups.push_back(g);
+        g = PlanGroup();
+    };
+    for (uint32_t li = 0; li < launches.size(); ++li) {
+        if (!eligible(launches[li])) {
+            close();
+            continue;
+        }
+        if (g.count && append(g, launches, li, max_taps)) continue;
+        close();
+        (void)append(g, launches, li, max_taps);
+    }
+    close();
+    return groups;
+}
+
+}
diff --git a/kanter_core_amd/csrc/replay_plan.h b/kanter_core_amd/csrc/replay_plan.h
--- /dev/null
+++ b/kanter_core_amd/csrc/replay_plan.h
@@ -0,0 +1,40 @@
+#pragma once
+#include <stddef.h>
+#include <stdint.h>
+
+#include <vector>
+
+namespace kc {
+
+enum { KC_PLAN_MAX_IN = 16, KC_PLAN_MAX_BATCH = 4, KC_PLAN_MAX_OPS = 16 };
+
+struct PlanLaunch {
+    uint32_t w = 0, h = 0;
+    int batch = 0;
+    bool flat_dense = false;
+    int start_src = -1;
+    uint32_t n_in = 0;
+    std::vector<uint32_t> words;
+    int in_from[KC_PLAN_MAX_BATCH][KC_PLAN_MAX_IN] = {};
+    int in_ch[KC_PLAN_MAX_BATCH][KC_PLAN_MAX_IN] = {};
+    const void *in_ptr[KC_PLAN_MAX_BATCH][KC_PLAN_MAX_IN] = {};
+};
+
+struct PlanGroup {
+    uint32_t first = 0, count = 0;
+    int start_src = -1;
+    uint32_t n_in = 0, n_ops = 0;
+    uint32_t tap_mask = 0;
+    uint32_t word[KC_PLAN_MAX_OPS] = {};
+    struct Rec {
+        uint32_t launch, index;
+        bool c_from_start;
+    } rec[KC_PLAN_MAX_OPS] = {};
+    struct In {
+        uint32_t launch, k;
+    } in[KC_PLAN_MAX_IN] = {};
+};
+
+std::vector<PlanGroup> replay_plan_taps(const std::vector<PlanLaunch> &launches, uint32_t max_taps);
+
+}
diff --git a/kanter_core_amd/csrc/specialize.cpp b/kanter_core_amd/csrc/specialize.cpp
--- a/kanter_core_amd/csrc/specialize.cpp
+++ b/kanter_core_amd/csrc/specialize.cpp
@@ -17,6 +17,7 @@
 extern const char kJitUpsampleH[];
 extern const char kJitUpsampleChainInc[];
 extern const char kJitChainPackH[] __attribute__((weak));
+extern const char kJitChainTapsH[] __attribute__((weak));
 
 namespace {
 
@@ -73,6 +74,7 @@
     uint32_t nt_mask = 0;
     uint32_t quads = 1;
     uint32_t in_tiers = 0;
+    uint32_t taps = 0;
     uint32_t word[KC_CHAIN_MAX_OPS] = {};
 
     std::string key() const
@@ -93,6 +95,10 @@
             k.push_back('t');
             k.append((const char *)&in_tiers, sizeof in_tiers);
         }
+        if (taps) {
+            k.push_back('T');
+            k.append((const char *)&taps, sizeof taps);
+        }
         return k;
     }
 };
@@ -164,7 +170,7 @@
     uint32_t h = 2166136261u;
     for (unsigned char c : s.key()) h = (h ^ c) * 16777619u;
     char buf[32];
-    std::snprintf(buf, sizeof buf, s.up_taps ? "kc_upchain_%08x" : "kc_chain_%08x", h);
+    std::snprintf(buf, sizeof buf, s.up_taps ? "kc_upchain_%08x" : s.taps ? "kc_tapchain_%08x" : "kc_chain_%08x", h);
     return buf;
 }
 
@@ -359,9 +365,61 @@
     return src;
 }
 
+static std::string generate_tapped(const Signature &s, int SPEC_WG)
+{
+    const char *taps_text = kJitChainTapsH;
+    if (!taps_text || !s.flat || s.up_taps || s.n_ops < 1 || s.n_ops > (uint32_t)KC_TAP_MAX_OPS) return std::string();
+    if (!(s.taps >> (s.n_ops - 1) & 1u) || (s.n_ops < 32 && s.taps >> s.n_ops) || __builtin_popcount(s.taps) > (int)KC_TAP_MAX) return std::string();
+    std::string src;
+    src.reserve(16384);
+    src += "namespace kc {\n";
+    src += kJitChainProgramH;
+    src += taps_text;
+    src += kPackedF4;
+    if (s.in_tiers) {
+        const char *pack_text = kJitChainPackH;
+        if (!pack_text) return std::string();
+        src += pack_text;
+    }
+    src += "}  // namespace kc\nusing namespace kc;\n";
+    char buf[256];
+    std::snprintf(buf, sizeof buf, "extern \"C\" __global__ __launch_bounds__(%d) void %s(const TapProgram P)\n{\n", SPEC_WG, kernel_name(s).c_str());
+    src += buf;
+    src += "    const unsigned int b = blockIdx.y;\n";
+    std::snprintf(buf, sizeof buf, "    const unsigned int col = blockIdx.x * %du + threadIdx.x;\n", SPEC_WG);
+    src += buf;
+    src += "    if (col >= P.rows * P.row_units) return;\n";
+    for (uint32_t k = 0; k < s.n_in; ++k) src += "    const f4 in" + std::to_string(k) + " = " + load_expr(s, k, "col") + ";\n";
+    src += "    const StepTableView pp{ P.step[b] };\n";
+    if (s.start_src < 0)
+        src += "    f4 acc = f4{ P.start_c[b], P.start_c[b], P.start_c[b], P.start_c[b] };\n";
+    else {
+        std::snprintf(buf, sizeof buf, "    f4 acc = in%d;\n", s.start_src);
+        src += buf;
+    }
+    uint32_t tap = 0;
+    for (uint32_t i = 0; i < s.n_ops; ++i) {
+        const uint32_t code = s.word[i] & 0xffu, from = (s.word[i] >> 8) & 0xffu;
+        if (code == CH_DIV_L || code == CH_DIV_R || code == CH_POW_L || code == CH_POW_R || code == CH_SAVE_LOAD || from > s.n_in) return std::string();
+        const std::string e = step_expr(s, i, "in", "");
+        if (e.empty()) return std::string();
+        src += "    acc = " + e + ";\n";
+        if (s.taps >> i & 1u) {
+            std::snprintf(buf, sizeof buf,
+                          s.nt_mask & 0x100u ? "    __builtin_nontemporal_store(acc.raw(), &reinterpret_cast<raw4 *>(P.tap[b][%u])[col]);\n"
+                                             : "    reinterpret_cast<raw4 *>(P.tap[b][%u])[col] = acc.raw();\n",
+                          tap++);
+            src += buf;
+        }
+    }
+    src += "}\n";
+    return src;
+}
+
 std::string generate(const Signature &s)
 {
     if (s.up_taps) return generate_up(s);
+    if (s.taps) return generate_tapped(s, spec_wg());
     const int SPEC_WG = spec_wg();
     bool pow = false;
     for (uint32_t i = 0; i < s.n_ops; ++i) pow |= (s.word[i] & 0xffu) == CH_POW_L || (s.word[i] & 0xffu) == CH_POW_R;
@@ -726,8 +784,10 @@
             std::fprintf(f, "{\"name\": \"%s\", \"n_in\": %u, \"start_src\": %d, \"flat\": %d, \"nt_mask\": %u, \"up_taps\": %u, \"up_wide\": %d, \"words\": [",
                          kernel_name(sig).c_str(), sig.n_in, sig.start_src, sig.flat ? 1 : 0, sig.nt_mask, sig.up_taps, sig.up_wide ? 1 : 0);
             for (uint32_t k = 0; k < sig.n_ops; ++k) std::fprintf(f, "%s%u", k ? ", " : "", sig.word[k]);
-            if (sig.in_tiers) std::fprintf(f, "], \"in_tiers\": %u}\n", sig.in_tiers);
-            else std::fprintf(f, "]}\n");
+            std::fprintf(f, "]");
+            if (sig.in_tiers) std::fprintf(f, ", \"in_tiers\": %u", sig.in_tiers);
+            if (sig.taps) std::fprintf(f, ", \"taps\": %u", sig.taps);
+            std::fprintf(f, "}\n");
             std::fclose(f);
         }
     }
@@ -797,6 +857,7 @@
     mix(s.nt_mask);
     mix(s.quads);
     mix(s.in_tiers);
+    mix(s.taps);
     for (uint32_t i = 0; i < s.n_ops; ++i) mix(s.word[i]);
     return h;
 }
@@ -804,7 +865,7 @@
 static bool same_signature(const Signature &a, const Signature &b)
 {
     return a.n_in == b.n_in && a.n_ops == b.n_ops && a.start_src == b.start_src && a.flat == b.flat && a.up_taps == b.up_taps &&
-           a.up_wide == b.up_wide && a.nt_mask == b.nt_mask && a.quads == b.quads && a.in_tiers == b.in_tiers &&
+           a.up_wide == b.up_wide && a.nt_mask == b.nt_mask && a.quads == b.quads && a.in_tiers == b.in_tiers && a.taps == b.taps &&
            std::memcmp(a.word, b.word, sizeof(uint32_t) * a.n_ops) == 0;
 }
 
@@ -895,6 +956,60 @@
         *launched = true;
         if (nt_mask) *nt_mask = sig.nt_mask;
         if (quads) *quads = sig.quads;
+        std::lock_guard<std::mutex> lk(spec().mu);
+        spec().launches++;
+    }
+    return e;
+}
+
+static Signature tapped_signature_of(const ChainProgram &P, uint32_t tap_mask)
+{
+    Signature sig = signature_of(P);
+    sig.quads = 1;
+    sig.in_tiers = 0;
+    sig.taps = tap_mask;
+    return sig;
+}
+
+static_assert(KC_TAP_MAX_OPS == (int)kQuadsMaxOps, "tapped programs are the short programs of chain_quads_for / pack_program_ok");
+
+hipError_t launch_chain_tapped(const ChainProgram &P, int batch, uint32_t tap_mask, float *const (*taps)[KC_TAP_MAX], hipStream_t s,
+                               bool *launched)
+{
+    *launched = false;
+    const uint64_t total = (uint64_t)P.rows * P.row_units;
+    if (P.rows != 1 || P.n_ops < 1 || P.n_ops > (uint32_t)KC_TAP_MAX_OPS || P.n_in > (uint32_t)KC_CHAIN_MAX_IN || total == 0 || total > 0xF0000000ull)
+        return hipSuccess;
+    if (!tap_mask || !(tap_mask >> (P.n_ops - 1) & 1u) || tap_mask >> P.n_ops || batch < 1 || batch > (int)KC_CHAIN_MAX_BATCH) return hipSuccess;
+    const Signature sig = tapped_signature_of(P, tap_mask);
+    hipFunction_t fn = spec_lookup(sig);
+    if (!fn) return hipSuccess;
+    static thread_local TapProgram T;
+    std::memset(&T, 0, sizeof T);
+    T.n_ops = P.n_ops;
+    T.n_in = P.n_in;
+    T.row_units = P.row_units;
+    T.rows = 1;
+    T.start_src = P.start_src;
+    T.nt_mask = sig.nt_mask;
+    T.tap_mask = tap_mask;
+    const uint32_t n_taps = (uint32_t)__builtin_popcount(tap_mask);
+    for (int b = 0; b < batch; ++b) {
+        for (uint32_t k = 0; k < P.n_in; ++k) T.in[b][k] = P.in[b][k];
+        T.start_c[b] = P.start_c[b];
+        for (uint32_t t = 0; t < n_taps; ++t) {
+            if (!taps[b][t]) return hipErrorInvalidValue;
+            T.tap[b][t] = taps[b][t];
+        }
+        std::memcpy(T.step[b], P.step[b], sizeof(ChainStepPair) * ((P.n_ops + 1) / 2));
+    }
+    size_t size = sizeof T;
+    const unsigned SPEC_WG = (unsigned)spec_wg();
+    void *extra[] = { HIP_LAUNCH_PARAM_BUFFER_POINTER, (void *)&T, HIP_LAUNCH_PARAM_BUFFER_SIZE, &size, HIP_LAUNCH_PARAM_END };
+    const unsigned gx = (unsigned)((total + SPEC_WG - 1) / SPEC_WG);
+    hipError_t e = hipModuleLaunchKernel(fn, gx, (unsigned)batch, 1, SPEC_WG, 1, 1, 0, s, nullptr, extra);
+    if (e == hipSuccess) {
+        *launched = true;
         std::lock_guard<std::mutex> lk(spec().mu);
         spec().launches++;
     }
@@ -1008,6 +1123,23 @@
     return rtc_compile(src, code, log) ? KC_OK : KC_ERR_GENERIC;
 }
 
+std::string specialize_source_tapped(const ChainProgram &P, uint32_t tap_mask) { return generate(tapped_signature_of(P, tap_mask)); }
+
+int specialize_compile_only_tapped(const ChainProgram &P, uint32_t tap_mask, std::string *log)
+{
+    if (!rtc().ok) {
+        *log = "libhiprtc not available";
+        return KC_ERR_UNSUPPORTED;
+    }
+    const std::string src = generate(tapped_signature_of(P, tap_mask));
+    if (src.empty()) {
+        *log = "not a tapped program";
+        return KC_ERR_INVALID_ARG;
+    }
+    std::vector<char> code;
+    return rtc_compile(src, code, log) ? KC_OK : KC_ERR_GENERIC;
+}
+
 int kernel_cache_set_dir(const char *dir)
 {
     DiskCache &d = disk();
@@ -1056,8 +1188,9 @@
 }
 
 int kernel_cache_precompile(const uint32_t *words, uint32_t n_ops, uint32_t n_in, int32_t start_src, bool flat, uint32_t nt_mask, uint32_t in_tiers,
-                            uint32_t up_taps, bool up_wide, const char *dir, std::string *log)
-{
+                            uint32_t up_taps, bool up_wide, const char *dir, std::string *log, uint32_t tap_mask)
+{
+    if (tap_mask && (!flat || up_taps || in_tiers)) return KC_ERR_INVALID_ARG;
     if (in_tiers && (!flat || up_taps || (n_in < 16 && in_tiers >> (2 * n_in)))) return KC_ERR_INVALID_ARG;
     for (uint32_t k = 0; k < n_in; ++k)
         if (KC_CHAIN_TIER(in_tiers, k) == 3u) return KC_ERR_INVALID_ARG;
@@ -1073,6 +1206,10 @@
     sig.in_tiers = in_tiers;
     for (uint32_t i = 0; i < n_ops; ++i) sig.word[i] = words[i];
     sig.quads = chain_quads_for(sig, 0);
+    if (tap_mask) {
+        sig.taps = tap_mask;
+        sig.quads = 1;
+    }
     const std::string src = generate(sig);
     if (src.empty()) {
         *log = "unknown step code";
```

Measured after the change: 7.113 million. No clear change (-0.3%).
